# ziwon-park/TRG-planner

Measured on AMD Instinct MI355X. Metric: TRG nodes+edges built/sec, higher is better.
Workload: dtype f32

## Files before the change

### include/trg_engine.h

```cpp
#ifndef TRG_ENGINE_H_
#define TRG_ENGINE_H_

#include <stddef.h>
#include <stdint.h>

#ifdef __cplusplus
extern "C" {
#endif

typedef struct TrgEngine TrgEngine;

typedef enum TrgStatus {
  TRG_OK = 0,
  TRG_ERR_INVALID_ARG = 1,
  TRG_ERR_NO_MAP = 2,
  TRG_ERR_NO_ROOT = 3,
  TRG_ERR_DEVICE = 4,
  TRG_ERR_NO_GRAPH = 5,
  TRG_ERR_NOT_FOUND = 6,
  TRG_ERR_IO = 7,
  TRG_ERR_CAPACITY = 8
} TrgStatus;

typedef enum TrgKind {
// ... 8 lines not shown
typedef struct TrgParams {
  int32_t is_verbose;
  float expand_dist;
  float robot_size;
  int32_t sample_num;
  float height_threshold;
  float collision_threshold;
  float update_collision_threshold;
  float safety_factor;
  float goal_tolerance;
} TrgParams;

typedef struct TrgSampler {
  uint32_t seed;
  int32_t table_bits;
} TrgSampler;

typedef struct TrgCsrView {
  int32_t num_nodes;
  int32_t num_edges;
  const float *node_xyz;
  const int32_t *node_state;
  const int32_t *rowptr;
  const int32_t *col;
  const float *weight;
  const float *dist;
  const int32_t *creation_id;
} TrgCsrView;

typedef struct TrgPathInfo {
  float direct_dist;
  float path_length;
  float avg_risk;
  int32_t num_points;
} TrgPathInfo;

typedef struct TrgStats {
  uint64_t map_points;
  uint64_t expanded_nodes;
  uint64_t trials;
  uint64_t samples;
  uint64_t created_nodes;
  uint64_t invalid_nodes;
  uint64_t edge_calls;
  uint64_t edge_evals_gpu;
  uint64_t nn_ties;
  uint64_t gate_uncertain;
  uint64_t sync_batches;
  uint64_t bytes_sample_kernel;
  uint64_t bytes_spec_kernel;
  uint64_t bytes_edge_kernel;
  uint64_t bytes_index_build;
  double ms_index_build;
  double ms_sample_kernel;
  double ms_spec_kernel;
  double ms_edge_kernel;
  uint64_t launches_sample_kernel;
  uint64_t launches_spec_kernel;
  uint64_t launches_edge_kernel;
  double ms_set_map_total;
  double ms_init_graph_total;
  double ms_replay_host;
  double ms_finalize_host;
  double ms_wait_gpu;
  uint64_t bfs_levels;
  uint64_t used_device_bfs;
  uint64_t bfs_fallbacks;
  uint64_t bfs_max_spin;
  uint64_t bfs_host_levels;
  uint64_t map_nn_ties;
  double ms_bfs_loop;
  double ms_deferred;
  uint64_t map_nn_resolved;
  uint64_t map_nn_unresolved;
  uint64_t bfs_tie_fixups;
  uint64_t bytes_spec_created;
  double ms_rare_events;
  uint64_t bfs_ticket_reruns;
  uint64_t bfs_multipass_rows;
  double ms_upload;
  uint64_t presampled_nodes;
  uint64_t stitch_gate_retries;
  uint64_t stitch_regrows;
} TrgStats;

TrgStatus trg_engine_create(const TrgParams *params, int device, TrgEngine **out);
void trg_engine_destroy(TrgEngine *e);
const char *trg_engine_last_error(const TrgEngine *e);
const char *trg_engine_device_arch(const TrgEngine *e);

TrgStatus trg_engine_set_global_map(TrgEngine *e, const float *xyz, size_t n, size_t stride);
TrgStatus trg_engine_set_global_map_device(TrgEngine *e, const float *d_xyz, size_t n, size_t stride);
TrgStatus trg_engine_set_local_map(TrgEngine *e, const float start_xy[2], const float *xyz, size_t n,
                                   size_t stride);
TrgStatus trg_engine_reset_map(TrgEngine *e, TrgKind kind);
TrgStatus trg_engine_reset_graph(TrgEngine *e, TrgKind kind);

TrgStatus trg_engine_init_graph(TrgEngine *e, const float start_xyz[3], const TrgSampler *sampler);
TrgStatus trg_engine_update_graph(TrgEngine *e);

TrgStatus trg_engine_export_csr(TrgEngine *e, TrgKind kind, TrgCsrView *out);
TrgStatus trg_engine_graph_sizes(TrgEngine *e, TrgKind kind, int32_t *num_nodes, int32_t *num_edges);
TrgStatus trg_engine_save_json(TrgEngine *e, const char *path);
TrgStatus trg_engine_load_json(TrgEngine *e, const char *path);

TrgStatus trg_engine_plan(TrgEngine *e, const float start_xy[2], const float goal_xyz[3],
                          float *path_xyz, int32_t max_points, TrgPathInfo *info);
TrgStatus trg_engine_plan_batch(TrgEngine *e, const float *starts_xy, const float *goals_xyz,
                                size_t m, float *path_xyz, int32_t path_cap, int32_t *offsets,
                                TrgPathInfo *infos);
int32_t trg_engine_check_reached(TrgEngine *e, const float pos_xy[2]);
int32_t trg_engine_check_replan(TrgEngine *e, const float pos_xy[2], const float *path_xyz,
                                int32_t n_path);
int32_t trg_engine_refine_path(const float *in_xyz, int32_t n_in, float *out_xyz, int32_t max_out);

TrgStatus trg_engine_is_collision_batch(TrgEngine *e, TrgKind map, float threshold, const float *xy,
                                        size_t m, int32_t *flag, int32_t *cnt, int32_t *n);
TrgStatus trg_engine_nearest_z_batch(TrgEngine *e, TrgKind map, const float *xy, size_t m, float *z);
TrgStatus trg_engine_edge_risk_batch(TrgEngine *e, TrgKind map, const float *p1_xyz,
                                     const float *p2_xyz, size_t m, int32_t *status, int32_t *n_pts,
                                     float *weight, float *dist);
TrgStatus trg_engine_is_frontier_batch(TrgEngine *e, const float *xy, size_t m, int32_t *flag);
typedef struct TrgPoseInfo {
  int32_t status, n_candidates, n_links;
  float z;
} TrgPoseInfo;
TrgStatus trg_engine_pose_links(TrgEngine *e, const float *poses_xy, int32_t m, float radius, int32_t cap,
                                int32_t *link_node, float *link_weight, float *link_dist, TrgPoseInfo *infos);

TrgStatus trg_engine_voxel_filter(TrgEngine *e, const float *xyz, size_t n, size_t stride, float leaf,
                                  float *out_xyz, size_t *n_out, int32_t *passthrough);

TrgStatus trg_engine_set_option(TrgEngine *e, const char *key, const char *value);
TrgStatus trg_engine_set_tile(TrgEngine *e, const float core_xyxy[4], uint32_t epoch);
typedef struct TrgBoundaryRec { int32_t local_id; float x, y, z; } TrgBoundaryRec;
typedef struct TrgCrossEdge { int32_t tile_a, id_a, tile_b, id_b; float weight, dist; } TrgCrossEdge;
TrgStatus trg_engine_stitch_boundary(TrgEngine *e, const float core_xyxy[4], int32_t cols, int32_t rows,
                                     int32_t tile, TrgBoundaryRec *d_rec, int32_t cap, int32_t *n_out);
TrgStatus trg_engine_stitch_cross(TrgEngine *e, int32_t tile, int32_t ntiles, const TrgBoundaryRec *d_all_rec,
                                  const int32_t *rec_offsets, TrgCrossEdge *d_edges, int32_t cap,
                                  int32_t *n_out);
TrgStatus trg_engine_stitch_assemble(TrgEngine *e, int32_t tile, int32_t ntiles, const int32_t *node_offsets,
                                     const TrgCrossEdge *d_all_edges, int32_t n_edges);
#define TRG_COMM_ID_BYTES 128
TrgStatus trg_engine_comm_unique_id(TrgEngine *e, uint8_t id[TRG_COMM_ID_BYTES]);
TrgStatus trg_engine_comm_init(TrgEngine *e, const uint8_t id[TRG_COMM_ID_BYTES], int32_t nranks, int32_t rank);
TrgStatus trg_engine_comm_adopt(TrgEngine *e, void *nccl_comm);
TrgStatus trg_engine_comm_join_local(TrgEngine *e, const char *group_name, int32_t nranks, int32_t rank);
TrgStatus trg_engine_comm_destroy(TrgEngine *e);
TrgStatus trg_engine_stitch_exchange(TrgEngine *e, const float core_xyxy[4], int32_t cols, int32_t rows,
                                     int32_t *n_boundary, int32_t *n_cross);
const char *trg_engine_fallback_reason(const TrgEngine *e);

typedef struct TrgFieldInfo {
  int32_t source;
  int32_t reached;
  int32_t rounds;
  int32_t host_syncs;
  double ms_device;
  double ms_total;
} TrgFieldInfo;
TrgStatus trg_engine_cost_field(TrgEngine *e, int32_t source_id, const float source_xy[2],
                                float *cost, int32_t *hops, int32_t *parent, TrgFieldInfo *info);
#define TRG_FIELD_BATCH_MAX 64
TrgStatus trg_engine_cost_field_batch(
    TrgEngine *e, int32_t m,
// ... 113 lines not shown
```

### trg-planner_amd/csrc/trg_bfs.inc

```

__device__ __forceinline__ int bfs_cell_x(const BfsDev &B, float x) {
  float t = floorf((x - B.gx0) * B.ginv);
  t = fminf(fmaxf(t, 0.0f), (float)(B.GW - 1));
  return (int)t;
}
__device__ __forceinline__ int bfs_cell_y(const BfsDev &B, float y) {
  float t = floorf((y - B.gy0) * B.ginv);
  t = fminf(fmaxf(t, 0.0f), (float)(B.GH - 1));
  return (int)t;
}
__device__ __forceinline__ float bfs_d2(float nx, float ny, float qx, float qy) {
  float acc = 0.0f;
  acc += (nx - qx) * (nx - qx);
  acc += (ny - qy) * (ny - qy);
  return acc;
}
__device__ __forceinline__ uint32_t bfs_hash(int key) { return fmix32((uint32_t)key * 0x9E3779B1u); }

__global__ __launch_bounds__(256) void k_bfs_insert_nodes(BfsDev B, int first, int count) {
  const int i = blockIdx.x * blockDim.x + threadIdx.x;
  if (i >= count) return;
  const int id = first + i;
  GridCell &c = B.gcell[bfs_cell_y(B, B.ny[id]) * B.GW + bfs_cell_x(B, B.nx[id])];
  const int pos = atomicAdd(&c.cnt, 1);
  if (pos < GRID_SLOTS) {
    c.id[pos] = id;
    c.x[pos] = B.nx[id];
    c.y[pos] = B.ny[id];
  } else {
    atomicOr(&B.ctrs[BFS_CTR_ERR], BFS_ERR_GRID_OVERFLOW);
  }
}

__device__ __forceinline__ int outcome_load(const int *p) {
  return __hip_atomic_load(p, __ATOMIC_RELAXED, __HIP_MEMORY_SCOPE_AGENT);
}
__device__ __forceinline__ void outcome_store(int *p, int v) {
  __hip_atomic_store(p, v, __ATOMIC_RELAXED, __HIP_MEMORY_SCOPE_AGENT);
}

#ifndef SPEC_WAVES_PER_SIMD
#define SPEC_WAVES_PER_SIMD 6
#endif
#ifndef SPEC3_WAVES_PER_SIMD
#define SPEC3_WAVES_PER_SIMD 5
#endif
#ifndef RESOLVE_EARLY_CREATE
#define RESOLVE_EARLY_CREATE 1
#endif
#ifndef TRG_RWV
#define TRG_RWV 8
#endif
constexpr int RW = TRG_RWV * 4;
static_assert(256 % RW == 0, "a commit workgroup covers whole resolve groups");

__global__ void k_bfs_clear_tie(BfsDev B) {
  if (threadIdx.x == 0) {
    atomicAnd(&B.ctrs[BFS_CTR_ERR], ~BFS_ERR_TIE);
    B.ctrs[BFS_CTR_NTIE] = 0;
  }
}

__global__ __launch_bounds__(256) void k_bfs_undo_slots(BfsDev B, int slots) {
  if (blockIdx.x == 0 && threadIdx.x == 0) B.stats64[STATS64_EXPAND_START] = 0ull;
  const int slot = blockIdx.x * blockDim.x + threadIdx.x;
  if (slot >= slots) return;
  const int o = B.c_outcome[slot];
  if (o != 3 && o != 4) return;
  const SlotRec &sr = B.slot_rec[slot];
  if ((sr.cls & SLOT_CLS_MASK) != 2) return;
  atomicSub(&B.gcell[bfs_cell_y(B, sr.y) * B.GW + bfs_cell_x(B, sr.x)].cnt, 1);
}

__global__ __launch_bounds__(QW *WAVE, EDGE_WAVES_PER_SIMD) void k_calls_gather(MapView m, QueryParams p, BfsDev B,
                                                           const int *list, int count,
                                                           const int *count_dev, DeviceCounters *ctr) {
  __shared__ EdgeLds lds;
  const int w = threadIdx.x >> 6;
  const int q = blockIdx.x * QW + w;
  if (count_dev) count = min(count, *count_dev);
  if (q >= count) return;
  const size_t at = (size_t)list[q];
  if (B.call_status[at] != CALL_PENDING) return;
  const int a = B.call_n1[at], b = B.call_n2[at];
  float *rec = B.mid + (size_t)q * MID_STRIDE;
  const EdgeMidOut o = edge_gather(m, p, B.nx[a], B.ny[a], B.nz[a], B.nx[b], B.ny[b], B.nz[b],
                                   lds.w[w], rec, ctr);
  store_mid(rec, o);
}

__global__ __launch_bounds__(256) void k_calls_finish(BfsDev B, const int *list, int count,
                                                      const int *count_dev, DeviceCounters *ctr) {
  __shared__ int wave_hits[4];
  const int q = blockIdx.x * blockDim.x + threadIdx.x;
  if (count_dev) count = min(count, *count_dev);
  const size_t at = (size_t)list[q < count ? q : 0];
  const bool live = q < count && B.call_status[at] == CALL_PENDING;
  const float *r = B.mid + (size_t)(live ? q : 0) * MID_STRIDE;
  const int h = wave_sum(live ? __float_as_int(r[MID_HITS]) : 0);
  if (lane_id() == 0) wave_hits[threadIdx.x >> 6] = h;
  __syncthreads();
  if (threadIdx.x == 0 && ctr) {
    const unsigned long long tot =
        (unsigned long long)(wave_hits[0] + wave_hits[1] + wave_hits[2] + wave_hits[3]);
    if (tot) atomicAdd(&ctr[blockIdx.x % COUNTER_SHARDS].edge_hits, tot);
  }
  if (!live) return;
  int st = __float_as_int(r[0]);
  float w = 0.0f;
  if ((st & EDGE_STATUS_MASK) == EDGE_OK) {
    float cov[3][3];
    mid_covariance(r, cov);
    int clamped = 0;
    w = risk_weight(cov, clamped);
    st |= clamped;
  }
  if (st & EDGE_GATE_UNCERTAIN) {
    const int k = atomicAdd(&B.ctrs[BFS_CTR_NUNC2], 1);
    if (k < BFS_UNC_CAP) {
      const int u = 2 * BFS_UNC_CAP + k;
      B.unc_list[u] = (int)at;
      B.unc_rec[3 * u] = B.nz[B.call_n1[at]];
      B.unc_rec[3 * u + 1] = B.nz[B.call_n2[at]];
      B.unc_rec[3 * u + 2] = r[2];
    }
  }
  B.call_status[at] = st & (EDGE_STATUS_MASK | EDGE_CLAMPED | EDGE_GATE_UNCERTAIN);
  B.call_w[at] = w;
  B.call_dist[at] = r[2];
}

__device__ __forceinline__ unsigned long long pair_key(int a, int b) {
  const unsigned lo = (unsigned)min(a, b), hi = (unsigned)max(a, b);
  return ((unsigned long long)lo << 32) | hi;
}
__device__ __forceinline__ uint32_t hash64(unsigned long long k) {
  return fmix32((uint32_t)(k >> 32) * 0x85EBCA6Bu ^ fmix32((uint32_t)k));
}

__global__ __launch_bounds__(256) void k_first_insert(FinDev F, BfsDev B, long long c0, long long ncalls,
                                                      int *sel_count) {
  if (blockIdx.x == 0 && threadIdx.x == 0) *sel_count = 0;
  const long long i = c0 + (long long)blockIdx.x * blockDim.x + threadIdx.x;
  if (i >= ncalls) return;
  F.call_slot[i] = -1;
  if (B.call_status[i] == CALL_NONE) return;
  int n2 = B.call_n2[i];
  if (n2 <= -2) {
    n2 = B.newid_of_call[-(long long)n2 - 2];
    B.call_n2[i] = n2;
  }
  const unsigned long long key = pair_key(B.call_n1[i], n2);
  const uint32_t mask = F.ht_size - 1u;
  uint32_t s = hash64(key) & mask;
  for (uint32_t probe = 0; probe < F.ht_size; ++probe) {
    const unsigned long long prev = atomicCAS(&F.ht_key[s], ~0ull, key);
    if (prev == ~0ull || prev == key) {
      atomicMin(&F.ht_seq[s], (int)i);
      F.call_slot[i] = (int)s;
      return;
    }
    s = (s + 1) & mask;
  }
  atomicOr(&B.ctrs[BFS_CTR_ERR], BFS_ERR_HASH);
}

__global__ __launch_bounds__(256) void k_calls_select_append(FinDev F, BfsDev B, long long c0, long long ncalls,
                                                             int *list, int *count, unsigned long long *total) {
  __shared__ int wave_cnt[4];
  __shared__ int wg_base;
  const long long i = c0 + (long long)blockIdx.x * blockDim.x + threadIdx.x;
  bool sel = false;
  if (i < ncalls && B.call_status[i] == CALL_PENDING) {
    const int slot = F.call_slot[i];
    sel = slot >= 0 && F.ht_seq[slot] == (int)i;
  }
  const unsigned long long m = ballot(sel);
  const int w = threadIdx.x >> 6;
  if (lane_id() == 0) wave_cnt[w] = __popcll(m);
  __syncthreads();
  if (threadIdx.x == 0) {
    const int tot = wave_cnt[0] + wave_cnt[1] + wave_cnt[2] + wave_cnt[3];
    if (tot) {
      wg_base = atomicAdd(count, tot);
      if (total) atomicAdd(total, (unsigned long long)tot);
    }
  }
  __syncthreads();
  if (!sel) return;
  int rank = __popcll(m & lanemask_lt());
  for (int k = 0; k < w; ++k) rank += wave_cnt[k];
// ... 205 lines not shown
```

### trg-planner_amd/csrc/trg_engine.cpp

```cpp
#include <hip/hip_runtime.h>
#include <math.h>

#include <algorithm>
#include <array>
#include <atomic>
#include <cstddef>
#include <chrono>
#include <cstdio>
#include <cstring>
#include <deque>
#include <fstream>
#include <functional>
#include <memory>
#include <optional>
#include <queue>
#include <sstream>
#include <string>
#include <thread>
#include <unordered_map>
#include <vector>

#include "../../include/trg_engine.h"
#include "abi_frame.h"
#include "graph_json.h"
// ... 435 lines not shown
struct TrgEngine {
  TrgEngine();
  ~TrgEngine();
  TrgParams prm{};
  int device = 0;
  int wall_clock_khz = 0;
  std::string err;
  std::string arch;
  bool device_ok = false;

  Stream s_main, s_edge;
  Stream s_aux;
  DevBuf<float> top_xy_d;
  Pinned<float> top_xy_h;
  Event top_ev;
  DevMap gmap, lmap;
  IndexScratch idx_scratch;
  DevBuf<DeviceCounters> d_ctr;
  DevBuf<unsigned> d_bounds;

  TrgSampler sampler{1, 16};
  std::vector<float> cos_t, sin_t;
  DevBuf<float> d_cos, d_sin;
  int table_bits_dev = 0;
  uint32_t epoch = 0;
  uint32_t epoch_base = 0;
  float core[4] = {-INFINITY, -INFINITY, INFINITY, INFINITY};

  enum GraphView { VIEW_POOL, VIEW_GRID, VIEW_KD_ORDER, VIEW_KD, VIEW_KDO, VIEW_CSR, VIEW_DEV_CSR, VIEW_UP_NODES,
                   VIEW_UP_EDGES, VIEW_STITCH_DEV, VIEW_COUNT };
  uint64_t graph_version = 1;
  uint64_t view_stamp[VIEW_COUNT] = {};
  bool current(GraphView v) const { return view_stamp[v] == graph_version; }
  std::vector<float> nx, ny, nz;
  std::vector<int> nstate;
  std::vector<int> ncid;
  int next_cid = 0;
  int node_id = 0;
  std::unordered_map<int, int> order_map;
  MapOrderSim nodes_sim;
  bool history_in_sim = false;
  std::vector<int> last_new2old;
  EdgePool edges;
  NodeGrid grid;
  std::vector<int> kd_insert_order;
  NodeKd kd;
  std::vector<float> kdo_x, kdo_y;
  std::vector<int> kdo_index;
  Csr csr_global;
  DevGraphUpload dev_up;
  Csr csr_stitched;
  int stitched_edges = 0;
  std::vector<int32_t> stitch_node_off;
  int stitch_tile = -1;
  uint64_t stitch_serial = 0;
  float root_pos[2] = {0, 0};
  float local_root[2] = {0, 0};
  std::unordered_map<int, int> local_map;
  std::vector<int> local_nodes;
  bool step3 = false;

  std::vector<int> queue;
  std::vector<CallRec> calls;
  static constexpr int NCHUNK = 3;
  static constexpr int CHUNK_MAX = 4096;
  Chunk chunks[NCHUNK];
  Chunk root_chunk;
  static constexpr int NEBATCH = 3;
  static constexpr int EBATCH_MAX = 1 << 16;
  EdgeBatch ebatches[NEBATCH];
  std::vector<int> pending_calls;

  PinnedBuf<float> sy_in, sy_in2, sy_f0, sy_f1;
  PinnedBuf<int> sy_i0, sy_i1, sy_i2;
  DevBuf<float> sy_mid;
  PinnedBuf<MapTieSet> mt_set;
  PinnedBuf<MapTieWalk> mt_walk;

  Csr csr_pre, csr_local;
  std::unique_ptr<StitchBufs> stitch;
  bool keep_preclean = false;
  bool use_device_bfs = true;
  bool defer_overlap = true;
  bool tail_overlap = true;
  PlanScratch plan_scratch;
  std::unique_ptr<Uploader> uploader;
  std::unique_ptr<ExchangeState> exchange;
  std::unique_ptr<FieldBufs> field;
  std::unique_ptr<TiledFieldBufs> tiled;
  double field_delta_scale = 4.0;
  enum { FIELD_MAP_NONE, FIELD_MAP_IDENTITY, FIELD_MAP_EXPLICIT } field_map_state = FIELD_MAP_NONE;
  std::vector<int> field_map;
  int debug_tie_every = 0;
  int debug_spec_bound = 0;
  int debug_fallback_level = -1;
  bool tie_inplace = true;
  int debug_lookback_level = -1;
  int debug_stall_level = -1;
  bool debug_wait_rerun = false;
  bool debug_call_stride = false;
  int resolve_tickets = 0;
  float gate_margin = 1e-4f;
  int debug_stitch_cap = 0;
  double comm_wait_seconds = 20.0;
  std::unique_ptr<BfsBuffers> bfs;
  std::string bfs_fallback_reason;
  uint64_t lv_hits_sample = 0, lv_hits_spec = 0;
  TrgStats stats{};

  int goal_node = -1;
  bool goal_known = false;
  float goal_pose2d[2] = {0, 0};

  TrgStatus fail(TrgStatus s, const std::string &m) {
    err = m;
    return s;
  }
};

namespace {

#define HIPCHK(e, expr)                                                                   \
  do {                                                                                    \
    hipError_t _err = (expr);                                                             \
    if (_err != hipSuccess) {                                                             \
      return (e)->fail(TRG_ERR_DEVICE, std::string(#expr) + ": " + hipGetErrorString(_err)); \
    }                                                                                     \
  } while (0)

enum EntryNeed { ENGINE, DEVICE };
template <typename Body>
TrgStatus entry(TrgEngine *e, const char *call, EntryNeed need, Body body) {
  if (!e) return TRG_ERR_INVALID_ARG;
  return abi_guard(call, [e](TrgStatus s, const std::string &m) { return e->fail(s, m); }, [&]() -> TrgStatus {
    if (need == DEVICE) {
      if (!e->device_ok) return e->fail(TRG_ERR_DEVICE, "engine has no usable device");
      if (hipSetDevice(e->device) != hipSuccess) return e->fail(TRG_ERR_DEVICE, "hipSetDevice failed");
    }
    return body();
  });
}

TrgStatus ensure_bytes(TrgEngine *e, DevArr &a, size_t need, bool keep = false) {
  if (a.p && a.bytes >= need) return TRG_OK;
  DevArr grown;
  HIPCHK(e, grown.reserve(std::max(need, a.bytes + a.bytes / 2)));
  if (keep && a.p && a.bytes) {
    hipError_t he = hipMemcpy(grown.p, a.p, a.bytes, hipMemcpyDeviceToDevice);
    if (he != hipSuccess) return e->fail(TRG_ERR_DEVICE, std::string("grow copy: ") + hipGetErrorString(he));
  }
  std::swap(a, grown);
  return TRG_OK;
}
TrgStatus ensure_all(TrgEngine *e, std::initializer_list<std::pair<DevArr *, size_t>> need) {
  for (const auto &n : need) {
    const TrgStatus st = ensure_bytes(e, *n.first, n.second);
    if (st != TRG_OK) return st;
  }
  return TRG_OK;
}

QueryParams qparams(const TrgEngine *e) {
  QueryParams q;
  q.robot_size = e->prm.robot_size;
  q.height_threshold = e->prm.height_threshold;
  q.collision_threshold = e->prm.collision_threshold;
  q.expand_dist = e->prm.expand_dist;
  q.sample_num = e->prm.sample_num;
  q.core_x0 = e->core[0];
  q.core_y0 = e->core[1];
  q.core_x1 = e->core[2];
  q.core_y1 = e->core[3];
  q.gate_margin = e->gate_margin;
  return q;
}

inline float key_to_float(unsigned k) {
  unsigned b = (k & 0x80000000u) ? (k & 0x7FFFFFFFu) : ~k;
  float f;
  memcpy(&f, &b, 4);
  return f;
}

#include "trg_engine_map.ipp"

TrgStatus ensure_sampler(TrgEngine *e, const TrgSampler *smp) {
  TrgSampler want = smp ? *smp : e->sampler;
  if (want.table_bits < 2 || want.table_bits > 20) want.table_bits = 16;
  e->sampler = want;
  if (e->table_bits_dev == want.table_bits && e->d_cos) return TRG_OK;
// ... 276 lines not shown
  if (e->arch.rfind("gfx950", 0) != 0) {
    return e->fail(TRG_ERR_DEVICE, "kernels are built for gfx950 only, device is " + e->arch);
  }
  HIPCHK(e, hipDeviceGetAttribute(&e->wall_clock_khz, hipDeviceAttributeWallClockRate, device));
  if (e->wall_clock_khz <= 0) return e->fail(TRG_ERR_DEVICE, "the device reports no wall-clock rate");
  HIPCHK(e, e->s_main.create());
  HIPCHK(e, e->s_edge.create_with_priority(0));
  HIPCHK(e, e->s_aux.create());
  HIPCHK(e, e->d_ctr.ensure(COUNTER_SHARDS));
  HIPCHK(e, hipMemset(e->d_ctr, 0, COUNTER_SHARDS * sizeof(DeviceCounters)));
  HIPCHK(e, e->d_bounds.ensure(4));
  e->step3 = (e->prm.expand_dist - e->prm.robot_size) < 0.25 * e->prm.expand_dist;
  e->bfs.reset(new BfsBuffers());
  e->uploader.reset(new Uploader());
  e->device_ok = true;
  if (const char *env = getenv("TRG_REPLAY")) e->use_device_bfs = std::string(env) != "host";
  reset_graph_global(e);
  return TRG_OK;
}

TrgStatus set_global_map(TrgEngine *e, const float *xyz, size_t n, size_t stride) {
  if ((n && !xyz) || stride < 3) return e->fail(TRG_ERR_INVALID_ARG, "bad map arguments");
  auto t0 = Clock::now();
  TrgStatus st = upload_and_build(e, e->gmap, xyz, n, stride);
  e->stats.ms_set_map_total = ms_since(t0);
  return st;
}

TrgStatus set_global_map_device(TrgEngine *e, const float *d_xyz, size_t n, size_t stride) {
  if ((n && !d_xyz) || stride < 3) return e->fail(TRG_ERR_INVALID_ARG, "bad map arguments");
  if (n == 0) {
    e->gmap.n = 0;
    e->gmap.valid = false;
    return TRG_OK;
  }
  return build_map(e, e->gmap, d_xyz, n, stride);
}

TrgStatus set_local_map(TrgEngine *e, const float start_xy[2], const float *xyz, size_t n, size_t stride) {
  if (!start_xy || (n && !xyz) || stride < 3) return e->fail(TRG_ERR_INVALID_ARG, "bad arguments");
  e->local_root[0] = start_xy[0];
  e->local_root[1] = start_xy[1];
  TrgStatus st = upload_and_build(e, e->lmap, xyz, n, stride);
  if (st != TRG_OK) return st;
  return set_local_graph(e);
}

TrgStatus reset_map(TrgEngine *e, TrgKind kind) {
  DevMap *m = pick_map(e, kind);
  m->top_wait();
  m->n = 0;
  m->valid = false;
  return TRG_OK;
}

TrgStatus reset_graph(TrgEngine *e, TrgKind kind) {
  if (kind == TRG_KIND_LOCAL) {
    e->local_nodes.clear();
    e->local_map.clear();
  } else {
    ensure_real_map(e);
    reset_graph_global(e);
    e->csr_global.clear();
    field_release(e);
  }
  return TRG_OK;
}

TrgStatus init_graph(TrgEngine *e, const float start_xyz[3], const TrgSampler *sampler) {
  if (!start_xyz) return e->fail(TRG_ERR_INVALID_ARG, "null start");
  if (!e->gmap.valid || e->gmap.n == 0) return e->fail(TRG_ERR_NO_MAP, "Map is empty");
  auto t_total = Clock::now();
  TrgStatus st = ensure_sampler(e, sampler);
  if (st != TRG_OK) return st;
  {
    TrgStats keep = e->stats;
    e->stats = TrgStats();
    e->stats.map_points = keep.map_points;
    e->stats.ms_index_build = keep.ms_index_build;
    e->stats.bytes_index_build = keep.bytes_index_build;
    e->stats.ms_set_map_total = keep.ms_set_map_total;
  }
  HIPCHK(e, hipMemsetAsync(e->d_ctr, 0, COUNTER_SHARDS * sizeof(DeviceCounters), e->s_main));
  e->lv_hits_sample = e->lv_hits_spec = 0;
  if (!e->use_device_bfs) ensure_real_map(e);
  MapOrderSim sim_before;
  if (e->use_device_bfs) {
    if (!e->history_in_sim) e->nodes_sim.adopt_bucket_state(e->order_map);
    sim_before = e->nodes_sim;
  }
  reset_graph_global(e);
  e->epoch = e->epoch_base;
  e->calls.clear();
  e->pending_calls.clear();
  e->csr_pre.clear();

  e->root_pos[0] = start_xyz[0];
  e->root_pos[1] = start_xyz[1];
  float rx = e->root_pos[0], ry = e->root_pos[1], rz = 0.0f;
  rx = rx + e->prm.expand_dist;
  int cnt = 0;
  for (;;) {
    float xy[2] = {rx, ry};
    int32_t flag = 1;
    st = collision_sync(e, e->gmap, e->prm.collision_threshold, xy, 1, &flag, nullptr, nullptr);
    if (st != TRG_OK) return st;
    if (!(rx >= e->core[0] && rx < e->core[2] && ry >= e->core[1] && ry < e->core[3])) flag = 1;
    if (!flag) {
      int32_t found = 0;
      st = nearest_z_sync(e, e->gmap, xy, 1, &rz, &found);
      if (st != TRG_OK) return st;
      break;
    }
    if (cnt > 100) return e->fail(TRG_ERR_NO_ROOT, "Failed to generate root node");
    const float u0 = sampler_uniform(e, 2 * cnt), u1 = sampler_uniform(e, 2 * cnt + 1);
    rx = rx + e->prm.expand_dist * u0;
    ry = ry + e->prm.expand_dist * u1;
    cnt++;
  }

  if (e->use_device_bfs) {
    st = build_graph_device(e, rx, ry, rz);
    if (st == TRG_OK) {
      read_counters(e);
      e->stats.used_device_bfs = 1;
      e->stats.ms_init_graph_total = ms_since(t_total);
      return TRG_OK;
    }
    if (e->bfs_fallback_reason.empty()) return st;
    e->stats.bfs_fallbacks++;
    HIPCHK(e, hipStreamSynchronize(e->s_main));
    HIPCHK(e, hipStreamSynchronize(e->s_edge));
    HIPCHK(e, hipMemset(e->d_ctr, 0, COUNTER_SHARDS * sizeof(DeviceCounters)));
    e->lv_hits_sample = e->lv_hits_spec = 0;
    e->nodes_sim = sim_before;
    ensure_real_map(e);
    reset_graph_global(e);
  }

  grid_rebuild(e);
  add_node_host(e, rx, ry, rz, TRG_NODE_VALID);
  st = expand_bfs(e, e->node_id - 1);
  if (st != TRG_OK) return st;
  auto t_fin = Clock::now();
  st = flush_pending(e, true);
  if (st != TRG_OK) return st;
  apply_calls(e, 0);
  if (e->keep_preclean) snapshot_csr(e, e->csr_pre);
  clean_graph(e);
  host_graph_changed(e);
  e->stats.ms_finalize_host = ms_since(t_fin);
  read_counters(e);
  e->stats.ms_init_graph_total = ms_since(t_total);
  return TRG_OK;
}

TrgStatus set_option(TrgEngine *e, const char *key, const char *value) {
  enum Kind {
    INT,
    BOOL,
    ZERO_OR_ONE,
    HOST_OR_DEVICE,
    FLOAT,
    POSITIVE_DOUBLE
  };
  const struct {
    const char *name;
    Kind kind;
    void *target;
  } options[] = {
      {"replay", HOST_OR_DEVICE, &e->use_device_bfs},
      {"defer_overlap", ZERO_OR_ONE, &e->defer_overlap},
      {"tail_overlap", ZERO_OR_ONE, &e->tail_overlap},
      {"tie_inplace", BOOL, &e->tie_inplace},
      {"keep_preclean", BOOL, &e->keep_preclean},
      {"resolve_tickets", INT, &e->resolve_tickets},
      {"field_delta_scale", POSITIVE_DOUBLE, &e->field_delta_scale},
      {"debug_gate_margin", FLOAT, &e->gate_margin},
      {"debug_tie_every", INT, &e->debug_tie_every},
      {"debug_spec_bound", INT, &e->debug_spec_bound},
      {"debug_stall_level", INT, &e->debug_stall_level},
      {"debug_lookback_level", INT, &e->debug_lookback_level},
      {"debug_fallback_level", INT, &e->debug_fallback_level},
      {"debug_call_stride", BOOL, &e->debug_call_stride},
      {"debug_wait_rerun", BOOL, &e->debug_wait_rerun},
      {"debug_stitch_cap", INT, &e->debug_stitch_cap},
      {"comm_wait_seconds", POSITIVE_DOUBLE, &e->comm_wait_seconds},
  };
  const std::string k(key), v(value);
  for (const auto &o : options) {
    if (k != o.name) continue;
    switch (o.kind) {
      case INT:
        *(int *)o.target = atoi(value);
        break;
      case BOOL:
        *(bool *)o.target = v != "0";
        break;
      case ZERO_OR_ONE:
        if (v != "0" && v != "1") return e->fail(TRG_ERR_INVALID_ARG, k + " must be 0 or 1");
        *(bool *)o.target = v == "1";
        break;
      case HOST_OR_DEVICE:
        if (v != "host" && v != "device") return e->fail(TRG_ERR_INVALID_ARG, k + " must be host or device");
        *(bool *)o.target = v == "device";
        break;
      case FLOAT:
        *(float *)o.target = (float)atof(value);
        break;
      case POSITIVE_DOUBLE: {
        const double d = strtod(value, nullptr);
        if (!(d > 0.0)) return e->fail(TRG_ERR_INVALID_ARG, k + " must be > 0");
        *(double *)o.target = d;
        break;
      }
    }
    return TRG_OK;
  }
  return e->fail(TRG_ERR_INVALID_ARG, "unknown option " + k);
}

TrgStatus set_tile(TrgEngine *e, const float core_xyxy[4], uint32_t epoch) {
  if (core_xyxy) {
    for (int i = 0; i < 4; ++i) e->core[i] = core_xyxy[i];
  } else {
    e->core[0] = e->core[1] = -INFINITY;
    e->core[2] = e->core[3] = INFINITY;
  }
  e->epoch_base = epoch;
  return TRG_OK;
}

TrgStatus is_frontier_batch(TrgEngine *e, const float *xy, size_t m, int32_t *flag);

TrgStatus update_graph(TrgEngine *e) {
  if (!e->gmap.valid) return e->fail(TRG_ERR_NO_MAP, "Map is empty");
  TrgStatus st = ensure_sampler(e, nullptr);
  if (st != TRG_OK) return st;
  e->epoch++;
  e->view_stamp[TrgEngine::VIEW_DEV_CSR] = 0;
  const size_t nodes_before = e->nx.size();
  const auto map_before = e->field_map_state;
  e->field_map_state = TrgEngine::FIELD_MAP_NONE;
  const bool trace_up = getenv("TRG_TIMING") != nullptr;
  auto t_up = Clock::now();
  auto lap_up = [&](const char *what) {
    if (trace_up) fprintf(stderr, "[trg update] %-28s %8.3f ms\n", what, ms_since(t_up));
  };
  ensure_pool(e);
  ensure_host_grid(e);
  ensure_kd_order(e);
  e->calls.clear();
  e->pending_calls.clear();
  lap_up("host structures ready");

  const size_t L = e->local_nodes.size();
// ... 512 lines not shown
```

### trg-planner_amd/csrc/trg_engine_bfs.inc

```

namespace {

struct LevelSet {
  DevArr node_rec;
  DevArr slot_rec;
  DevArr c_outcome;
  DevArr lv_hash;
  DevArr resc;
  void apply(BfsDev &B) const {
    B.node_rec = (NodeRec *)node_rec.p;
    B.slot_rec = (SlotRec *)slot_rec.p;
    B.c_outcome = (int *)c_outcome.p;
    B.lv_hash = (HashEnt *)lv_hash.p;
    B.resc = use_resc ? (RescueRec *)resc.p : nullptr;
  }
  bool use_resc = false;
};

constexpr int H_CLEAN_TOTALS = 32;
constexpr int H_ROUND2_CALLS = 34;
constexpr int H_STEP3_LEFT = 40;
constexpr int H_STATS64 = 64;
constexpr int H_CTRS_WORDS = 96;
static_assert(BFS_CTR_COUNT <= H_CLEAN_TOTALS && H_CLEAN_TOTALS + 2 <= H_ROUND2_CALLS &&
                  H_ROUND2_CALLS < H_STEP3_LEFT && H_STEP3_LEFT < H_STATS64 && H_STATS64 % 2 == 0 &&
                  H_STATS64 + 32 <= H_CTRS_WORDS,
              "pinned words overlap");

enum : int {
  S64_DEF_KEPT = 5, S64_MAX_SPIN, S64_MULTIPASS, S64_DRAWS, S64_SAMPLES, S64_DISC_HITS, S64_SPEC_HITS,
  S64_CANDIDATES, S64_PARENT_HITS, S64_EXPAND_START = STATS64_EXPAND_START, S64_EXPAND_TICKS = STATS64_EXPAND_TICKS,
  S64_PHASES = 16, S64_WORDS = 16 + 1024 * 8
};
static_assert(S64_PARENT_HITS < S64_EXPAND_START && S64_EXPAND_START < S64_EXPAND_TICKS && S64_EXPAND_TICKS < S64_PHASES,
              "report_stats fetches the words in front of S64_PHASES");

struct BfsBuffers {
  BfsDev B{};
  FinDev F{};
  LevelSet lv[2];
  DevArr nx, ny, nz, nstate, gcell, ncov, nexp, nhits, front0, front1, fxy0, fxy1;
  DevArr mid, unc_list, unc_rec, mt_rec, ctrs, stats64, wg_state, c_cell, tl, scan_tmp, s3_scratch;
  DevArr call_n1, call_n2, call_status, call_w, call_dist, newid_of_call, call_slot;
  DevArr sel_list, def_counts;
  DevArr ht_key, ht_seq, ok_seq, deg, fill, rowptr, col, seq, w, dist;
  DevArr map_order, keep_flag, keep_pos, new2old, old2new, deg_new, rowptr_new, col2, w2, dist2, xyz2, state2;
  Pinned<int> h_ctrs;
  int stamp_serial = 0;
  std::vector<int> hm_state;
  std::vector<float> hm_x, hm_y;
  std::vector<int> rp_stamp, rp_head;
  int rp_serial = 0;
  unsigned long long nodes_created = 0, nodes_invalid = 0;
};

TrgStatus mirror_nodes(TrgEngine *e, BfsBuffers &bb, int n) {
  const size_t at = bb.hm_state.size();
  if ((size_t)n <= at) return TRG_OK;
  const size_t k = (size_t)n - at;
  bb.hm_state.resize(n);
  bb.hm_x.resize(n);
  bb.hm_y.resize(n);
  HIPCHK(e, hipMemcpy(bb.hm_state.data() + at, bb.B.nstate + at, k * sizeof(int), hipMemcpyDeviceToHost));
  HIPCHK(e, hipMemcpy(bb.hm_x.data() + at, bb.B.nx + at, k * sizeof(float), hipMemcpyDeviceToHost));
  HIPCHK(e, hipMemcpy(bb.hm_y.data() + at, bb.B.ny + at, k * sizeof(float), hipMemcpyDeviceToHost));
  return TRG_OK;
}

inline float ref_d2(float x, float y, float qx, float qy) {
  float acc = 0;
  acc += (x - qx) * (x - qx);
  acc += (y - qy) * (y - qy);
  return acc;
}

struct Nearest {
  int nn = -1;
  float best = INFINITY;
  std::vector<int> tied;
  void start(const BfsBuffers &bb, const SlotRec &sr, int V0) {
    nn = sr.nn0;
    best = nn >= 0 ? sr.d0sq : INFINITY;
    tied.clear();
    if (nn >= 0 && (sr.cls & SLOT_TIE)) {
      for (int i = 0; i < V0; ++i)
        if (ref_d2(bb.hm_x[i], bb.hm_y[i], sr.x, sr.y) == best) tied.push_back(i);
    } else if (nn >= 0) {
      tied.push_back(nn);
    }
  }
  void offer(const BfsBuffers &bb, int id, float qx, float qy) {
    const float dd = ref_d2(bb.hm_x[id], bb.hm_y[id], qx, qy);
    if (dd < best) {
      best = dd;
      nn = id;
      tied.assign(1, id);
    } else if (dd == best) {
      tied.push_back(id);
    }
  }
  bool tie() const { return tied.size() > 1; }
  int winner(const BfsBuffers &bb, int V_at, float qx, float qy) {
    if (!tie()) return nn;
    std::sort(tied.begin(), tied.end());
    return kd_tie_winner(bb.hm_x.data(), bb.hm_y.data(), V_at, qx, qy, tied);
  }
};

constexpr int BFS_FCAP = 1 << 16;
constexpr int CALL_EVAL_BATCH = 1 << 22;
constexpr int BFS_ERR_SOFT = BFS_ERR_TIE | BFS_ERR_STALL | BFS_ERR_TIE_CLS;
constexpr long long DEF_BATCH_MIN = 6000;

std::string err_text(int code) {
  std::string t;
  if (code & BFS_ERR_GRID_OVERFLOW) t += "grid-cell overflow;";
  if (code & BFS_ERR_NB_OVERFLOW) t += "neighbour list overflow;";
  if (code & BFS_ERR_VCAP) t += "node capacity;";
  if (code & BFS_ERR_TIE) t += "exact fp32 distance tie (kd-tree order decides);";
  if (code & BFS_ERR_TIE_CLS) t += "exact fp32 distance tie among pre-level nodes;";
  if (code & BFS_ERR_HASH) t += "hash table full;";
  if (code & BFS_ERR_LEVEL_TOO_BIG) t += "BFS level too large;";
  if (code & BFS_ERR_CLEAN) t += "clean remap;";
  if (code & BFS_ERR_STALL) t += "resolve stalled;";
// ... 344 lines not shown
    float t = std::floor((v - v0) * B.ginv);
    t = std::min(std::max(t, 0.0f), (float)(n - 1));
    return (int)t;
  };
  std::vector<int> call_n1(slots), call_n2(slots, -1), call_st(slots, CALL_NONE), next_front;
  std::vector<float> call_w(slots, 0.0f), call_d(slots, 0.0f);
  Nearest near;
  int Vcur = V0;
  unsigned long long invalid = 0;
  for (int qpos = 0; qpos < lv.mcur; ++qpos) {
    const int u = front[qpos];
    for (int j = 0; j < S; ++j) {
      const size_t slot = (size_t)qpos * S + j;
      call_n1[slot] = u;
      if (j >= nrec[qpos].n_acc) continue;
      const SlotRec &sr = srec[slot];
      const float qx = sr.x, qy = sr.y;
      near.start(bb, sr, V0);
      {
        const float rad = (near.nn >= 0 ? std::sqrt(near.best) : e->prm.expand_dist * 1.01f) * 1.001f + 1e-6f;
        const int cx0 = cell_xy(qx - rad, B.gx0, B.GW), cx1 = cell_xy(qx + rad, B.gx0, B.GW);
        const int cy0 = cell_xy(qy - rad, B.gy0, B.GH), cy1 = cell_xy(qy + rad, B.gy0, B.GH);
        for (int cy = cy0; cy <= cy1; ++cy)
          for (int cx = cx0; cx <= cx1; ++cx) {
            const size_t cell = (size_t)cy * B.GW + cx;
            if (bb.rp_stamp[cell] != serial) continue;
            for (int id = bb.rp_head[cell]; id >= 0; id = rp_next[id - V0]) near.offer(bb, id, qx, qy);
          }
      }
      if (near.nn < 0) return e->fail(TRG_ERR_DEVICE, "host level replay: a sample without a nearest node");
      if (near.tie()) e->stats.nn_ties++;
      const int nn = near.winner(bb, Vcur, qx, qy);
      if (bb.hm_state[nn] == TRG_NODE_INVALID) continue;
      if (std::sqrt(near.best) < e->prm.robot_size) {
        if (nn != u) {
          call_n2[slot] = nn;
          call_st[slot] = CALL_PENDING;
        }
        continue;
      }
      if ((sr.cls & SLOT_CLS_MASK) != 2)
        return e->fail(TRG_ERR_DEVICE, "host level replay: missing speculative edge");
      const bool ok = (sr.status & EDGE_STATUS_MASK) == EDGE_OK;
      const int id = Vcur++;
      new_hits.push_back(sr.hits);
      bb.hm_x.push_back(qx);
      bb.hm_y.push_back(qy);
      bb.hm_state.push_back(ok ? TRG_NODE_VALID : TRG_NODE_INVALID);
      new_z.push_back(sr.z);
      {
        const size_t cell = (size_t)cell_xy(qy, B.gy0, B.GH) * B.GW + cell_xy(qx, B.gx0, B.GW);
        rp_next.push_back(bb.rp_stamp[cell] == serial ? bb.rp_head[cell] : -1);
        bb.rp_stamp[cell] = serial;
        bb.rp_head[cell] = id;
      }
      NodeCov nc{};
      if (ok) {
        call_n2[slot] = id;
        call_st[slot] = sr.status & EDGE_STATUS_MASK;
        call_d[slot] = sr.dist;
        next_front.push_back(id);
        if (sr.w_given) nc.cov[0] = sr.cov[0];
        nc.w_given = sr.w_given;
        nc.call = (int)(lv.call_base + (long long)slot);
      } else {
        invalid++;
      }
      new_cov.push_back(nc);
    }
  }
  const int created = Vcur - V0;
  bb.nodes_created += (unsigned long long)created;
  bb.nodes_invalid += invalid;
  if (Vcur > B.vcap || (int)next_front.size() > B.fcap)
    return e->fail(TRG_ERR_CAPACITY, "host level replay: capacity");
  if (created > 0) {
    const size_t at = (size_t)V0, n = (size_t)created;
    HIPCHK(e, hipMemcpy(B.nx + at, bb.hm_x.data() + at, n * sizeof(float), hipMemcpyHostToDevice));
    HIPCHK(e, hipMemcpy(B.ny + at, bb.hm_y.data() + at, n * sizeof(float), hipMemcpyHostToDevice));
    HIPCHK(e, hipMemcpy(B.nz + at, new_z.data(), n * sizeof(float), hipMemcpyHostToDevice));
    HIPCHK(e, hipMemcpy(B.nstate + at, bb.hm_state.data() + at, n * sizeof(int), hipMemcpyHostToDevice));
    HIPCHK(e, hipMemcpy(B.ncov + at, new_cov.data(), n * sizeof(NodeCov), hipMemcpyHostToDevice));
    HIPCHK(e, hipMemcpy(B.nhits + at, new_hits.data(), n * sizeof(int), hipMemcpyHostToDevice));
    launch_bfs_insert_nodes(B, V0, created, s);
  }
  if (!next_front.empty()) {
    HIPCHK(e, hipMemcpy(B.front_next, next_front.data(), next_front.size() * sizeof(int),
                        hipMemcpyHostToDevice));
    std::vector<float> fxy(2 * next_front.size());
    for (size_t k = 0; k < next_front.size(); ++k) {
      fxy[2 * k] = bb.hm_x[next_front[k]];
      fxy[2 * k + 1] = bb.hm_y[next_front[k]];
    }
    HIPCHK(e, hipMemcpy(B.fxy_next, fxy.data(), fxy.size() * sizeof(float), hipMemcpyHostToDevice));
  }
  const size_t cb = (size_t)lv.call_base;
  HIPCHK(e, hipMemcpy(B.call_n1 + cb, call_n1.data(), slots * sizeof(int), hipMemcpyHostToDevice));
  HIPCHK(e, hipMemcpy(B.call_n2 + cb, call_n2.data(), slots * sizeof(int), hipMemcpyHostToDevice));
  HIPCHK(e, hipMemcpy(B.call_status + cb, call_st.data(), slots * sizeof(int), hipMemcpyHostToDevice));
  HIPCHK(e, hipMemcpy(B.call_w + cb, call_w.data(), slots * sizeof(float), hipMemcpyHostToDevice));
  HIPCHK(e, hipMemcpy(B.call_dist + cb, call_d.data(), slots * sizeof(float), hipMemcpyHostToDevice));
  int ctr_host[BFS_CTR_COUNT] = {0};
  ctr_host[BFS_CTR_V] = Vcur;
  ctr_host[BFS_CTR_MNEXT] = (int)next_front.size();
  HIPCHK(e, hipMemcpy(B.ctrs, ctr_host, BFS_CTR_NUNC2 * sizeof(int), hipMemcpyHostToDevice));
  HIPCHK(e, hipStreamSynchronize(s));
  lv.v_after = Vcur;
  lv.mnext = (int)next_front.size();
  lv.replayed = true;
  e->stats.bfs_host_levels++;
  return TRG_OK;
}

TrgStatus Build::repair_level(Level &lv) {
  TrgStatus st;
  if (e->step3 && lv.n_unc > 0)
    return fallback("a slope gate left to the host's libm in a build with expandGraph's step 3");
  if (CS > 1 && ((lv.err & BFS_ERR_SOFT & ~BFS_ERR_STALL) || lv.n_mt > 0))
    return fallback("exact fp32 distance tie in a build with expandGraph's step 3");
  const auto t_rare = Clock::now();
  const bool any_rare = lv.n_mt > 0 || lv.n_unc > 0 || (lv.err & (BFS_ERR_SOFT | BFS_ERR_LOOKBACK));
  constexpr int ERR_WAIT = BFS_ERR_STALL | BFS_ERR_LOOKBACK;
  if ((lv.err & ERR_WAIT) && !(lv.err & ~(BFS_ERR_SOFT | ERR_WAIT))) {
    const int hook = e->debug_wait_rerun ? ((lv.err & BFS_ERR_LOOKBACK) ? 2 : 1) : 0;
    e->stats.bfs_ticket_reruns++;
    st = redo_commit(lv, false, true, hook);
    if (st == TRG_ERR_CAPACITY) e->stats.ms_rare_events += ms_since(t_rare);
    if (st != TRG_OK) return st;
  }
  if (lv.err & ~BFS_ERR_SOFT) {
    if (any_rare) e->stats.ms_rare_events += ms_since(t_rare);
    return fallback(err_text(lv.err));
  }
  if (lv.n_mt > 0 && (st = fix_map_ties(lv)) != TRG_OK) return st;
  if (lv.n_unc > 0) {
    void *status = (char *)B.slot_rec + offsetof(SlotRec, status);
    if ((st = resolve_uncertain(lv.n_unc, status, sizeof(SlotRec), lv.parity, lv.unc_ctr)) != TRG_OK) return st;
    if (unc_changed && (st = (lv.err & BFS_ERR_SOFT) ? undo_level(lv) : redo_commit(lv)) != TRG_OK) return st;
  }
  if ((lv.err & BFS_ERR_SOFT) == BFS_ERR_TIE_CLS && !lv.undone && (st = fix_pre_level_ties(lv)) != TRG_OK)
    return st;
  if ((lv.err & BFS_ERR_SOFT) == BFS_ERR_TIE && !lv.undone && e->tie_inplace && !debug_tie_level(e, lv.index)) {
    if ((st = settle_ties_in_place(lv)) != TRG_OK) return st;
  }
  if (lv.err & BFS_ERR_SOFT) {
    if (CS > 1) return fallback("a level of a build with expandGraph's step 3 needs the host replay");
    if (!lv.undone && (st = undo_level(lv)) != TRG_OK) return st;
    if ((st = replay_level(lv)) != TRG_OK) return st;
  }
  if (any_rare) {
    e->stats.ms_rare_events += ms_since(t_rare);
    if (getenv("TRG_TRACE_LEVELS"))
      fprintf(stderr, "[trg bfs] level %d: rare events (map ties %d, uncertain gates %d, err %d%s) took %.3f ms\n",
              lv.index, lv.n_mt, lv.n_unc, lv.err, lv.replayed ? ", host replay" : "",
              ms_since(t_rare));
  }
  return TRG_OK;
}

TrgStatus Build::allocate() {
  const float pad = e->prm.expand_dist * 2 + e->prm.robot_size;
  float cell = e->prm.robot_size;
  if (!(cell > 0)) return fallback("robot_size <= 0");
  const double ex = (double)(m.bounds[2] - m.bounds[0]) + 2 * pad + 4 * cell;
  const double ey = (double)(m.bounds[3] - m.bounds[1]) + 2 * pad + 4 * cell;
  if ((ex / cell + 2) * (ey / cell + 2) > 256e6) return fallback("node grid too large");
  B.gx0 = m.bounds[0] - pad - 2 * cell;
  B.gy0 = m.bounds[1] - pad - 2 * cell;
  B.gcell_size = cell;
  B.ginv = 1.0f / cell;
  B.GW = (int)floor(ex / cell) + 2;
  B.GH = (int)floor(ey / cell) + 2;
  const size_t ncell = (size_t)B.GW * B.GH;
  const double vbound = ex * ey / (0.8660254 * cell * cell) * 1.05 + 4096;
  if (vbound > 400e6) return fallback("node capacity bound too large");
  const size_t vcap = (size_t)vbound;
  const size_t fcap = BFS_FCAP;
  const size_t slots = fcap * (size_t)std::max(S, 1);

  if (!level_kernels_support(qp, cell))
    return fallback("sample_num or expand_dist / robot_size outside the level kernels' range");
  TrgStatus st;
  const size_t wg_words = slots / 16 + 64 + 8;
  const size_t I = sizeof(int), FL = sizeof(float);
  if ((st = ensure_all(e, {{&bb.nx, vcap * FL}, {&bb.ny, vcap * FL}, {&bb.nz, vcap * FL}, {&bb.nstate, vcap * I},
                           {&bb.gcell, ncell * sizeof(GridCell)}, {&bb.ncov, vcap * sizeof(NodeCov)},
                           {&bb.front0, fcap * I}, {&bb.front1, fcap * I}, {&bb.fxy0, fcap * sizeof(float2)},
                           {&bb.fxy1, fcap * sizeof(float2)}})) != TRG_OK)
    return st;
  B.nx = (float *)bb.nx.p;
  B.ny = (float *)bb.ny.p;
  B.nz = (float *)bb.nz.p;
  B.nstate = (int *)bb.nstate.p;
  B.vcap = (int)std::min<size_t>(vcap, 0x7FFFFFF0);
  B.gcell = (GridCell *)bb.gcell.p;
  B.ncov = (NodeCov *)bb.ncov.p;
  B.front_cur = (int *)bb.front0.p;
  B.front_next = (int *)bb.front1.p;
  B.fxy_cur = (float2 *)bb.fxy0.p;
  B.fxy_next = (float2 *)bb.fxy1.p;
  B.fcap = (int)fcap;
  const size_t ht_need = hash_size(fcap, std::max(S, 1));
  for (LevelSet &l : bb.lv) {
    if ((st = ensure_all(e, {{&l.node_rec, fcap * sizeof(NodeRec)}, {&l.slot_rec, slots * sizeof(SlotRec)},
                             {&l.c_outcome, slots * I}, {&l.lv_hash, ht_need * sizeof(HashEnt)}})) != TRG_OK)
      return st;
    l.use_resc = e->step3;
    if (e->step3 && (st = ensure_bytes(e, l.resc, slots * sizeof(RescueRec))) != TRG_OK) return st;
    HIPCHK(e, hipMemsetAsync(l.lv_hash.p, 0, ht_need * sizeof(HashEnt), s));
  }
  if ((st = ensure_all(e, {{&bb.mid, edge_mid_floats(CALL_EVAL_BATCH) * FL},
                           {&bb.unc_list, (3 * BFS_UNC_CAP + BFS_TIE_CAP) * I},
                           {&bb.unc_rec, 3 * 3 * BFS_UNC_CAP * FL}, {&bb.mt_rec, 2 * MAPTIE_CAP * sizeof(MapTieRec)},
                           {&bb.ctrs, BFS_CTR_COUNT * I}, {&bb.stats64, S64_WORDS * sizeof(unsigned long long)},
                           {&bb.wg_state, wg_words * sizeof(unsigned long long)},
                           {&bb.c_cell, slots * sizeof(unsigned long long)}, {&bb.nexp, vcap * sizeof(int4)},
                           {&bb.nhits, vcap * I}, {&bb.scan_tmp, (std::max(slots, vcap) / 2048 + 8) * I}})) != TRG_OK)
    return st;
  B.mid = (float *)bb.mid.p;
  B.unc_list = (int *)bb.unc_list.p;
  B.tie_list = B.unc_list + 3 * BFS_UNC_CAP;
  B.unc_rec = (float *)bb.unc_rec.p;
  B.mt_rec = (MapTieRec *)bb.mt_rec.p;
  B.ctrs = (int *)bb.ctrs.p;
  B.stats64 = (unsigned long long *)bb.stats64.p;
  B.wg_state = (unsigned long long *)bb.wg_state.p;
  HIPCHK(e, hipMemsetAsync(B.wg_state, 0, wg_words * sizeof(unsigned long long), s));
  B.ticket = (unsigned *)(B.wg_state + (slots / 16 + 64));
  ticket_base = 0;
  B.tl = nullptr;
  if (getenv("TRG_TIMELINE")) {
    const size_t tl_bytes = (size_t)(1 << 16) * 12 * 6 * sizeof(unsigned long long);
    if ((st = ensure_bytes(e, bb.tl, tl_bytes)) != TRG_OK) return st;
    B.tl = (unsigned long long *)bb.tl.p;
    HIPCHK(e, hipMemsetAsync(B.tl, 0, tl_bytes, s));
  }
  B.c_cell = (unsigned long long *)bb.c_cell.p;
  HIPCHK(e, hipMemsetAsync(B.c_cell, 0, slots * sizeof(unsigned long long), s));
  B.nexp = (int4 *)bb.nexp.p;
  B.nhits = (int *)bb.nhits.p;
  if (!bb.h_ctrs) {
    HIPCHK(e, bb.h_ctrs.ensure(H_CTRS_WORDS, hipHostMallocMapped | hipHostMallocCoherent));
    memset(bb.h_ctrs, 0, H_CTRS_WORDS * sizeof(int));
  }
  {
    void *dp = nullptr;
    HIPCHK(e, hipHostGetDevicePointer(&dp, bb.h_ctrs, 0));
    B.host_ctrs = (int *)dp;
  }

  bb.hm_state.clear();
  bb.hm_x.clear();
  bb.hm_y.clear();
  bb.nodes_created = bb.nodes_invalid = 0;
  HIPCHK(e, hipMemsetAsync(B.gcell, 0, ncell * sizeof(GridCell), s));
  HIPCHK(e, hipMemsetAsync(B.ctrs, 0, BFS_CTR_COUNT * sizeof(int), s));
  HIPCHK(e, hipMemsetAsync(B.stats64, 0, S64_WORDS * sizeof(unsigned long long), s));

  calls_bound = std::min<size_t>(vcap * (size_t)std::max(S, 1) * (size_t)CS, 0x7FFFFFF0u);
  fht = 1024;
  while ((unsigned long long)fht < (unsigned long long)calls_bound && fht < (1u << 31)) fht <<= 1;
  if ((st = ensure_all(e, {{&bb.ht_key, fht * sizeof(unsigned long long)}, {&bb.ht_seq, fht * I},
                           {&bb.ok_seq, fht * I}, {&bb.def_counts, 2 * I}})) != TRG_OK)
    return st;
  F.ht_key = (unsigned long long *)bb.ht_key.p;
  F.ht_seq = (int *)bb.ht_seq.p;
  F.ok_seq = (int *)bb.ok_seq.p;
  F.ht_size = fht;
  overlap = !e->step3 && e->defer_overlap;
  if (overlap) {
    HIPCHK(e, hipMemsetAsync(F.ht_key, 0xFF, (size_t)fht * sizeof(unsigned long long), s));
    HIPCHK(e, hipMemsetAsync(F.ht_seq, 0x7F, (size_t)fht * sizeof(int), s));
  }
  HIPCHK(e, hipMemsetAsync(F.ok_seq, 0x7F, (size_t)fht * sizeof(int), s));
  s_def = overlap ? e->s_edge : s;
  return TRG_OK;
// ... 370 lines not shown
    if ((st = read_ctrs()) != TRG_OK) return st;
    if (bb.h_ctrs[BFS_CTR_ERR]) return fallback(err_text(bb.h_ctrs[BFS_CTR_ERR]));
    e->nx.clear();
    e->ny.clear();
    e->nz.clear();
    e->nstate.clear();
    e->ncid.clear();
  }
  lap("clean kernels + CSR to host");
  e->node_id = Vn;
  lap("host graph state");
  e->history_in_sim = true;
  if (Vn > 0) graph_changed(e, {TrgEngine::VIEW_CSR, TrgEngine::VIEW_DEV_CSR});
  else graph_changed(e, {TrgEngine::VIEW_CSR});
  return TRG_OK;
}

TrgStatus Build::report_stats() {
  unsigned long long s64[S64_PHASES];
  memcpy(s64, bb.h_ctrs + H_STATS64, sizeof(s64));
  if (getenv("TRG_DEBUG_STATS")) {
    std::vector<int> hs(V), hx(4 * (size_t)V);
    HIPCHK(e, hipMemcpy(hs.data(), B.nstate, (size_t)V * sizeof(int), hipMemcpyDeviceToHost));
    HIPCHK(e, hipMemcpy(hx.data(), B.nexp, (size_t)V * 16, hipMemcpyDeviceToHost));
    unsigned long long d = 0, a = 0;
    size_t zero = 0;
    for (int i = 0; i < V; ++i)
      if (hs[i] != -1) {
        d += (unsigned long long)hx[4 * (size_t)i + 1];
        a += (unsigned long long)(hx[4 * (size_t)i] & 0xFF);
        zero += hx[4 * (size_t)i + 1] == 0;
      }
    fprintf(stderr, "[trg stats] device draws %llu samples %llu | host sum draws %llu samples %llu | valid nodes with 0 draws %zu\n",
            s64[S64_DRAWS], s64[S64_SAMPLES], d, a, zero);
  }
  if (B.tl) {
    constexpr int UNITS = 1 << 16, KINDS = 12, TAGS = 6;
    std::vector<unsigned long long> tl((size_t)UNITS * KINDS * TAGS);
    HIPCHK(e, hipMemcpy(tl.data(), B.tl, tl.size() * sizeof(unsigned long long), hipMemcpyDeviceToHost));
    static const char *names[KINDS] = {"sample start", "sample end", "spec start", "spec end", "resolve start",
                                       "resolve collected", "resolve decided(w0)", "resolve published",
                                       "(unused)", "(unused)", "commit start", "commit sums known"};
    for (int t = 0; t < TAGS; ++t) {
      const unsigned long long *base = &tl[(size_t)t * UNITS * KINDS];
      unsigned long long t0 = ~0ull;
      for (int i = 0; i < UNITS; ++i)
        if (base[i]) t0 = std::min(t0, base[i]);
      if (t0 == ~0ull) continue;
      fprintf(stderr, "[trg timeline] level attempt +%d (us after its first sampling workgroup started; n, min, p10, median, p90, max):\n", t);
      for (int k = 0; k < KINDS; ++k) {
        std::vector<double> v;
        for (int i = 0; i < UNITS; ++i)
          if (base[(size_t)k * UNITS + i]) v.push_back(((double)base[(size_t)k * UNITS + i] - (double)t0) / 100.0);
        if (v.empty()) continue;
        std::sort(v.begin(), v.end());
        auto q = [&](double f) { return v[(size_t)(f * (v.size() - 1))]; };
        fprintf(stderr, "[trg timeline]   %-22s n=%6zu  %8.1f %8.1f %8.1f %8.1f %8.1f%s\n", names[k], v.size(), q(0), q(0.1), q(0.5),
                q(0.9), q(1), k >= 4 ? "   (of the PREVIOUS level's resolve launch)" : "");
      }
    }
  }
  if (getenv("TRG_PHASE_TIMING") && ncalls > 0) {
    std::vector<unsigned long long> ph(1024 * 8);
    HIPCHK(e, hipMemcpy(ph.data(), B.stats64 + S64_PHASES, ph.size() * sizeof(unsigned long long), hipMemcpyDeviceToHost));
    double t[8] = {0};
    for (size_t i = 0; i < ph.size(); ++i) t[i & 7] += (double)ph[i];
    const double nodes = (double)(ncalls / std::max(S * CS, 1));
    if (getenv("TRG_PHASE_TIMING")[0] == 'r')
      fprintf(stderr, "[trg resolve phases, cycles per workgroup] collect %.0f  decide(wave 0) %.0f  records+stash %.0f  other waves %.0f  look-back %.0f\n",
              t[0] / nodes * (32.0 / S), t[1] / nodes * (32.0 / S), t[2] / nodes * (32.0 / S), t[3] / nodes * (32.0 / S), t[4] / nodes * (32.0 / S));
    else
    fprintf(stderr, "[trg expand phases, cycles per node] sample: tile %.0f  nodegrid %.0f  sampling %.0f  classify %.0f  hash %.0f  record %.0f | spec (per node): tile %.0f  edges %.0f\n",
            t[0] / nodes, t[1] / nodes, t[2] / nodes, t[3] / nodes, t[4] / nodes, t[5] / nodes, t[6] / nodes, t[7] / nodes);
  }
  e->stats.expanded_nodes = (uint64_t)(ncalls / std::max(S * CS, 1));
  e->stats.trials = s64[S64_DRAWS];
  e->stats.samples = s64[S64_SAMPLES];
  e->stats.created_nodes = bb.nodes_created + 1;
  e->stats.invalid_nodes = bb.nodes_invalid;
  e->stats.edge_calls = s64[S64_SAMPLES];
  e->stats.edge_evals_gpu = s64[S64_CANDIDATES] + s64[S64_DEF_KEPT];
  e->lv_hits_sample = s64[S64_DISC_HITS];
  e->lv_hits_spec = s64[S64_SPEC_HITS];
  e->stats.bytes_spec_created = 12ull * s64[S64_PARENT_HITS];
  e->stats.ms_finalize_host = ms_since(t_fin);
  e->stats.bfs_levels = (uint64_t)levels;
  e->stats.bfs_max_spin = s64[S64_MAX_SPIN];
  e->stats.ms_sample_kernel += (double)s64[S64_EXPAND_TICKS] / (double)e->wall_clock_khz;
  e->stats.bfs_multipass_rows = s64[S64_MULTIPASS];
  return TRG_OK;
}

TrgStatus build_graph_device(TrgEngine *e, float root_x, float root_y, float root_z) {
  e->bfs_fallback_reason.clear();
  Build b(e);
  b.B.cstride = b.CS;
  TrgStatus st;
  if ((st = b.allocate()) != TRG_OK) return st;
  if ((st = b.seed_root(root_x, root_y, root_z)) != TRG_OK) return st;
  if ((st = b.level_loop()) != TRG_OK) return st;
  if ((st = b.finish_deferred()) != TRG_OK) return st;
  if ((st = b.assemble_csr()) != TRG_OK) return st;
  if ((st = b.clean_and_fetch()) != TRG_OK) return st;
  return b.report_stats();
}

}
```

### trg-planner_amd/csrc/trg_kernels.h

```cpp
#pragma once
#include <hip/hip_runtime.h>
#include <stdint.h>

namespace trg {

struct MapView {
  const float *x;
  const float *y;
  const float *z;
  const int *perm;
  const float4 *pt;
  const int *cell_start;
  float x0, y0;
  float inv_g;
  int W, H;
  int n;
};

constexpr int MAPTIE_CAP = 256;
constexpr int MAPTIE_SET_CAP = 16;
struct MapTieRec {
  int slot;
  float qx, qy;
  float d2;
};
struct MapTieSet {
  int count;
  float d2;
  int sidx[MAPTIE_SET_CAP];
  int perm[MAPTIE_SET_CAP];
  float x[MAPTIE_SET_CAP], y[MAPTIE_SET_CAP], z[MAPTIE_SET_CAP];
};

struct QueryParams {
  float robot_size;
  float height_threshold;
  float collision_threshold;
  float expand_dist;
  int sample_num;
  float core_x0, core_y0, core_x1, core_y1;
  float gate_margin;
};

enum : int {
  EDGE_OK = 0,
  EDGE_GATE = 1,
  EDGE_SEG = 2,
  EDGE_EMPTY = 3,
  EDGE_FEW = 4,
  EDGE_STATUS_MASK = 7,
  EDGE_GATE_UNCERTAIN = 8,
  EDGE_CLAMPED = 16,
};

constexpr int COUNTER_SHARDS = 64;
struct alignas(128) DeviceCounters {
  unsigned long long sample_hits;
  unsigned long long edge_hits;
  unsigned long long spec_hits;
  unsigned long long nn_ties;
  unsigned long long overflow;
  unsigned long long pad[11];
};

void launch_init_bounds(unsigned *d_bounds, hipStream_t s);
void launch_bounds(const float *d_xyz, size_t n, size_t stride, unsigned *d_bounds, hipStream_t s);
void launch_cell_count(const float *d_xyz, size_t n, size_t stride, float x0, float y0, float inv_g,
                       int W, int H, int *d_cell_of, int *d_rank, int *d_counts, hipStream_t s);
hipError_t voxel_grid_filter(const float *d_xyz, size_t n, size_t stride, float leaf, float *d_out,
                             size_t *n_out, int *status, hipStream_t s);
void launch_exclusive_scan(const int *d_counts, int *d_out, int m, int *d_tmp, hipStream_t s);
bool index_bins_plan(size_t n, size_t ncell, int *bin_shift, int *nbins, int *nwg);
void launch_index_bins(const float *d_xyz, size_t n, size_t stride, float x0, float y0, float inv_g, int W, int H,
                       int ncell, int bin_shift, int nbins, int nwg, int *d_hist, int *d_base, int *d_tmp,
                       float4 *d_scratch_a, float4 *d_scratch_b, int *d_cell_start, float *x, float *y, float *z,
                       int *perm, float4 *pt, hipStream_t s);
void launch_scatter_sort_aos(const float *d_xyz, size_t n, size_t stride, const int *d_cell_of,
                             const int *d_rank, int ncell, const int *d_cell_start, void *d_aos, float *x,
                             float *y, float *z, int *perm, float4 *pt, hipStream_t s);

void launch_probe_collision(const MapView &m, QueryParams p, float threshold, const float *d_xy,
                            int count, int *flag, int *cnt, int *n, DeviceCounters *ctr,
                            hipStream_t s);
void launch_probe_nearest_z(const MapView &m, QueryParams p, const float *d_xy, int count, float *z,
                            int *found, DeviceCounters *ctr, hipStream_t s);
void launch_edges(const MapView &m, QueryParams p, const float *d_p1, const float *d_p2, int count,
                  float *mid, int *status, int *n_pts, float *weight, float *dist,
                  DeviceCounters *ctr, hipStream_t s);
size_t edge_mid_floats(size_t edges);

void launch_sample_nodes(const MapView &m, QueryParams p, const float *cos_t, const float *sin_t,
                         int table_bits, uint32_t seed, uint32_t epoch, const float *node_xy,
                         const int *node_id, int count, int *n_acc, int *n_draws, float *sx,
                         float *sy, float *sz, DeviceCounters *ctr, int *mt_count,
                         MapTieRec *mt_rec, hipStream_t s);
void launch_map_tied_set(const MapView &m, float qx, float qy, float r0, MapTieSet *d_out,
                         hipStream_t s);
struct MapTieWalk {
  unsigned long long key;
  float lo[2], hi[2];
  int cur_perm;
  int axis;
  float qx, qy;
  int aperm, bperm;
  float ax, ay, bx, by;
  int done;
  int first;
  int steps;
  int ticket;
};
void launch_map_tie_walk(const MapView &m, MapTieWalk *d_state, int grid_steps, int block_steps, hipStream_t s);
void launch_collect_first(const MapView &m, int M, float *d_out_xy, hipStream_t s);
void launch_spec_edges(const MapView &m, QueryParams p, const float *node_xyz, int count,
                       const int *n_acc, const float *sx, const float *sy, const float *sz,
                       float *mid, int *status, int *n_pts, float *weight, float *dist,
                       DeviceCounters *ctr, hipStream_t s);

constexpr int GRID_SLOTS = 4;
constexpr int BFS_TIE_CAP = 64;
constexpr int BFS_UNC_CAP = 4096;
enum : int {
  BFS_CTR_V = 0, BFS_CTR_MNEXT = 1, BFS_CTR_NCAND = 2, BFS_CTR_NUNC = 3, BFS_CTR_ERR = 4,
  BFS_CTR_DONE = 5,
  BFS_CTR_NTIE = 5,
  BFS_CTR_NMAPTIE = 6 ,
  BFS_CTR_NUNC1 = 8,
  BFS_CTR_NUNC2 = 14,
  BFS_CTR_COUNT = 16
};
enum : int {
  BFS_ERR_GRID_OVERFLOW = 1, BFS_ERR_NB_OVERFLOW = 2, BFS_ERR_VCAP = 4, BFS_ERR_TIE = 8,
  BFS_ERR_HASH = 16, BFS_ERR_LEVEL_TOO_BIG = 32, BFS_ERR_CLEAN = 64,
  BFS_ERR_STALL = 128,
  BFS_ERR_LOOKBACK = 512,
  BFS_ERR_STEP3 = 1024,
  BFS_ERR_TIE_CLS = 256
};
enum : int { CALL_NONE = -2, CALL_PENDING = -1 };

struct alignas(64) GridCell {
  int cnt;
  int id[GRID_SLOTS];
  float x[GRID_SLOTS], y[GRID_SLOTS];
  int pad[3];
};
struct alignas(16) SlotRec {
  float x, y, z;
  float d0sq;
  int nn0;
  int cls;
  int status;
  float dist;
  float cov[6];
  int w_given;
  int hits;
};
enum : int { SLOT_CLS_MASK = 0xFF, SLOT_TIE = 0x100 };
struct alignas(16) NodeRec {
  int n_acc, n_draws;
  int hits_sample, hits_spec;
  unsigned cand_lo, cand_hi;
  int pad1[2];
  float px, py, pz;
  int pad2;
};
struct alignas(16) HashEnt {
  unsigned long long tagcell;
  int slot;
  int pad;
  float x, y;
  int pad2[2];
};
constexpr int RESC_MAX = 14;
struct alignas(16) RescueRec {
  int pre;
  int n;
  int slot[RESC_MAX];
};
struct alignas(16) NodeCov {
  float cov[6];
  int w_given;
  int call;
};

struct BfsDev {
  float *nx, *ny, *nz;
  int *nstate;
  NodeCov *ncov;
  int vcap;
  GridCell *gcell;
  float gx0, gy0, ginv, gcell_size;
  int GW, GH;
  int *front_cur, *front_next;
  float2 *fxy_cur, *fxy_next;
  int fcap;
  NodeRec *node_rec;
  SlotRec *slot_rec;
  int *c_outcome;
  unsigned long long *c_cell;
  HashEnt *lv_hash;
  int ht_size;
  RescueRec *resc;
  unsigned long long *wg_state;
  unsigned *ticket;
  int4 *nexp;
  int *nhits;
  float *mid;
  int *unc_list;
  float *unc_rec;
  int *tie_list;
  MapTieRec *mt_rec;
  int *call_n1, *call_n2, *call_status;
  float *call_w, *call_dist;
  int *newid_of_call;
  int cstride;
  int *ctrs;
  int *host_ctrs;
  unsigned long long *stats64;
  unsigned long long *tl;
};
constexpr int STATS64_EXPAND_START = 14, STATS64_EXPAND_TICKS = 15;

struct FinDev {
  unsigned long long *ht_key;
  int *ht_seq;
  int *ok_seq;
  unsigned ht_size;
  int *call_slot;
  int *deg, *fill, *rowptr;
  int *col, *seq;
  float *w, *dist;
};

void launch_bfs_insert_nodes(const BfsDev &B, int first, int count, hipStream_t s);
void launch_bfs_clear_tie(const BfsDev &B, hipStream_t s);
void launch_bfs_undo_slots(const BfsDev &B, int slots, hipStream_t s);
constexpr int LEVEL_MAX_SAMPLES = 64;
constexpr int LEVEL_STEP3_STRIDE = 16;
void launch_level_expand(const MapView &m, QueryParams p, const float *cos_t, const float *sin_t,
                         int table_bits, uint32_t seed, uint32_t epoch, const BfsDev &B, int count,
                         const int *count_dev, int node_base, int parity, int tag, int pub_stamp,
                         DeviceCounters *ctr, hipStream_t s, int which = 3);
bool level_kernels_support(const QueryParams &p, float grid_cell);
void launch_level_resolve_commit(const BfsDev &B, QueryParams p, int count, int new_state,
                                 long long call_base, int V0, int tag, int epoch, hipStream_t s,
                                 int stall_test,
                                 bool ticketed, unsigned *ticket_base);
typedef int TrgStatus_t;
TrgStatus_t launch_step3_calls(const BfsDev &B, int V, float range, int *scratch, int *h_left, hipStream_t s);
void launch_bfs_stats(const BfsDev &B, int V, unsigned long long *out, hipStream_t s);
void launch_node_cov(const MapView &m, QueryParams p, const BfsDev &B, int v_lo, int v_hi, hipStream_t s);
void launch_node_weights(const BfsDev &B, int V, hipStream_t s);
void launch_calls_eval(const MapView &m, QueryParams p, const BfsDev &B, const int *list, int count,
                       const int *count_dev, DeviceCounters *ctr, hipStream_t s);
void launch_first_insert(const FinDev &F, const BfsDev &B, long long c0, long long c1, int *sel_count,
                         hipStream_t s);
void launch_calls_select_append(const FinDev &F, const BfsDev &B, long long c0, long long c1, int *list,
                                int *count, unsigned long long *total, hipStream_t s);
void launch_calls_select2_append(const FinDev &F, const BfsDev &B, long long ncalls, int *list, int *count,
                                 unsigned long long *total, hipStream_t s);
void launch_fin_insert_count(const FinDev &F, const BfsDev &B, long long ncalls, hipStream_t s);
void launch_fin_scatter(const FinDev &F, const BfsDev &B, long long ncalls, hipStream_t s);
void launch_fin_rowsort(const FinDev &F, int V, hipStream_t s);
void launch_fin_clean(const FinDev &F, const BfsDev &B, const int *map_order, int V, int *keep_flag,
                      int *keep_pos, int *new2old, int *old2new, int *deg_new, int *rowptr_new,
                      int *scan_tmp, int *col, float *w, float *dist, float *xyz, int *state,
                      hipStream_t s);
void launch_fin_clean_weights(const FinDev &F, const BfsDev &B, int V, const int *keep_pos, const int *new2old,
                              const int *rowptr_new, float *w, hipStream_t s);

struct StitchRec {
  int id;
  float x, y, z;
};
struct StitchEdge {
  int tile_a, id_a, tile_b, id_b;
  float weight, dist;
};
constexpr int STITCH_MAX_TILES = 64;
void launch_stitch_boundary(const float *d_xyz, int V, const float core[4], int sides, float d, int *flag,
                            int *off, int *scan_tmp, StitchRec *rec, int cap, hipStream_t s);
void launch_stitch_pairs(const StitchRec *all, const int *rec_offsets, int tile, int ntiles, float d,
                         int pass, int *cnt, const int *off, int *pair_a, int *pair_b, hipStream_t s);
void launch_stitch_pair_points(const StitchRec *all, const int *pair_a, const int *pair_b, int n,
                               float *p1, float *p2, hipStream_t s);
void launch_stitch_edge_select(const StitchRec *all, const int *rec_offsets, int tile, int ntiles,
                               const int *pair_a, const int *pair_b, const int *status,
                               const float *weight, const float *dist, int n, int *flag, int *off,
                               int *scan_tmp, int *n_unc, StitchEdge *out, int cap, hipStream_t s);
void launch_stitch_assemble(const StitchEdge *edges, int n_edges, int tile, int ntiles,
                            const int *node_offsets, const int *rowptr, const int *col, const float *w,
                            const float *dist, int V, int *extra, int *deg, int *rowptr_new,
                            int *scan_tmp, int *fill, int *col_new, float *w_new, float *dist_new,
                            int phase, hipStream_t s);

constexpr unsigned long long FIELD_KEY_NONE = ~0ull;
constexpr unsigned FIELD_EDGE_SKIP = 0xFFFFFFFFu;
constexpr int FIELD_NODE_INVALID = -1;
constexpr int FIELD_MAX_SOURCES = 64;
struct alignas(128) FieldEdgeStats {
  double sum;
  int count;
  int bad;
};
// ... 133 lines not shown
```

### trg-planner_amd/csrc/trg_kernels.hip

```cpp
#include "trg_kernels.h"

#include <float.h>
#include <limits.h>
#include <type_traits>

namespace trg {

namespace {

constexpr int WAVE = 64;
constexpr int HCAP = 1024;

__device__ __forceinline__ int lane_id() { return threadIdx.x & (WAVE - 1); }

__device__ __forceinline__ unsigned long long lanemask_lt() {
  return (1ull << lane_id()) - 1ull;
}

__device__ __forceinline__ unsigned long long ballot(bool pred) {
  return __builtin_amdgcn_ballot_w64(pred);
}

__device__ __forceinline__ void wave_lds_sync() {
  __builtin_amdgcn_fence(__ATOMIC_RELEASE, "wavefront");
// ... 349 lines not shown
        if (q >= p) continue;
        const float threshold = fmaxf(FLT_MIN, precision * max_diag);
        if (fabsf(W[p][q]) > threshold || fabsf(W[q][p]) > threshold) {
          finished = false;
          Rot jl, jr;
          jacobi_2x2(W, p, q, jl, jr);
          rows_rotate(W, p, q, jl);
          cols_rotate(U, p, q, rot_t(jl));
          cols_rotate(W, p, q, jr);
          max_diag = fmaxf(max_diag, fmaxf(fabsf(W[p][p]), fabsf(W[q][q])));
        }
      }
    }
  }
  float sv[3];
#pragma unroll
  for (int i = 0; i < 3; ++i) {
    const float a = fabsf(W[i][i]);
    sv[i] = a;
    if (a != 0.0f) {
      const float sgn = W[i][i] / a;
#pragma unroll
      for (int r = 0; r < 3; ++r) U[r][i] *= sgn;
    }
  }
#pragma unroll
  for (int i = 0; i < 3; ++i) sv[i] *= scale;
#pragma unroll
  for (int i = 0; i < 3; ++i) {
    int pos = i;
    float mx = sv[i];
#pragma unroll
    for (int k2 = 0; k2 < 3; ++k2) {
      if (k2 > i && sv[k2] > mx) {
        mx = sv[k2];
        pos = k2;
      }
    }
    if (mx == 0.0f) break;
    if (pos != i) {
      const float ts = sv[i];
      sv[i] = sv[pos];
      sv[pos] = ts;
#pragma unroll
      for (int r = 0; r < 3; ++r) {
        const float tu = U[r][i];
        U[r][i] = U[r][pos];
        U[r][pos] = tu;
      }
    }
  }
}

__device__ float risk_weight(const float cov[3][3], int &clamped) {
  float U[3][3];
  svd_u3(cov, U);
  float fro = 0.0f;
#pragma unroll
  for (int cc = 0; cc < 3; ++cc)
#pragma unroll
    for (int r = 0; r < 3; ++r) fro += U[r][cc] * U[r][cc];
  float e20 = U[2][0], e21 = U[2][1];
  if (fro > 0.0f) {
    const float nrm = sqrtf(fro);
    e20 = e20 / nrm;
    e21 = e21 / nrm;
  }
  float hor = e20, ver = e21;
  if (hor < 0.0f) hor = -e20;
  if (ver < 0.0f) ver = -e21;
  const float ratio = 0.8f;
  float w = ratio * hor + (1 - ratio) * ver;
  clamped = 0;
  if ((double)w < 0.1) {
    w = 0.0f;
    clamped = EDGE_CLAMPED;
  }
  return w;
}

constexpr int MID_STRIDE = 24;
constexpr int MID_HITS = 3;
constexpr int MID_MOMENTS = 4;

struct EdgeGeom {
  float dist, dirx, diry, cx, cy;
  int uncertain;
  bool gated;
};

__device__ __forceinline__ EdgeGeom edge_geometry(const QueryParams &p, float x1, float y1, float z1,
                                                  float x2, float y2, float z2) {
  EdgeGeom g;
  const float ex = x1 - x2, ey = y1 - y2;
  g.dist = sqrtf(ex * ex + ey * ey);
  g.uncertain = 0;
  g.gated = false;
  const double lhs = (double)fabsf(z1 - z2) * (double)p.robot_size;
  const double rhs = (double)p.height_threshold * (double)g.dist;
  const double margin = (double)p.gate_margin;
  if (lhs > rhs * (1.0 + margin)) {
    g.gated = true;
  } else if (!(lhs < rhs * (1.0 - margin))) {
    g.uncertain = EDGE_GATE_UNCERTAIN;
  }
  const float dx = x2 - x1, dy = y2 - y1;
  const float sq = dx * dx + dy * dy;
  g.dirx = dx;
  g.diry = dy;
  if (sq > 0.0f) {
    const float nrm = sqrtf(sq);
    g.dirx = dx / nrm;
    g.diry = dy / nrm;
  }
  const float half = 0.5f * g.dist;
  g.cx = x1 + half * g.dirx;
  g.cy = y1 + half * g.diry;
  return g;
}

struct Moments {
  double s_x = 0, s_y = 0, s_z = 0, s_xx = 0, s_xy = 0, s_xz = 0, s_yy = 0, s_yz = 0, s_zz = 0;
  int kept = 0, in_range = 0;
};

struct EllipseParams {
  float cx, cy, a2, bb, aabb, r00, r01, r10, r11, z_ref;
  bool is_circle;
};

__device__ __forceinline__ bool ellipse_point(const EllipseParams &ep, float px, float py, float pz,
                                              Moments &mo) {
  const float ddx = px - ep.cx, ddy = py - ep.cy;
  const float d2 = ddx * ddx + ddy * ddy;
  bool keep = false;
  if (d2 <= ep.a2) {
    mo.in_range++;
    const float X = ep.r00 * ddx + ep.r01 * ddy;
    const float Y = ep.r10 * ddx + ep.r11 * ddy;
    keep = ep.is_circle;
    if (!ep.is_circle) keep = (X * X) * ep.bb + (Y * Y) * ep.a2 < ep.aabb;
    if (keep) {
      mo.kept++;
      const double xd = (double)X, yd = (double)Y, zd = (double)pz - (double)ep.z_ref;
      mo.s_x += xd;
      mo.s_y += yd;
      mo.s_z += zd;
      mo.s_xx += xd * xd;
      mo.s_xy += xd * yd;
      mo.s_xz += xd * zd;
      mo.s_yy += yd * yd;
      mo.s_yz += yd * zd;
      mo.s_zz += zd * zd;
    }
  }
  return keep;
}

struct EllipseCounts {
  int kept = 0, in_range = 0;
};
__device__ __forceinline__ bool ellipse_point(const EllipseParams &ep, float px, float py, float ,
                                              EllipseCounts &mo) {
  const float ddx = px - ep.cx, ddy = py - ep.cy;
  const float d2 = ddx * ddx + ddy * ddy;
  bool keep = false;
// ... 243 lines not shown
  cov[1][2] = cov[2][1] = (float)((sm[7] - n * my * mz) * inv);
  cov[2][2] = (float)((sm[8] - n * mz * mz) * inv);
}

__device__ __forceinline__ void reduce_store_moments(WaveTile &t, const Moments &mo, float *rec) {
  const int lane = lane_id();
  double *P = (double *)&t;
  wave_lds_sync();
  P[0 * MOM_STRIDE + lane] = mo.s_x;
  P[1 * MOM_STRIDE + lane] = mo.s_y;
  P[2 * MOM_STRIDE + lane] = mo.s_z;
  P[3 * MOM_STRIDE + lane] = mo.s_xx;
  P[4 * MOM_STRIDE + lane] = mo.s_xy;
  P[5 * MOM_STRIDE + lane] = mo.s_xz;
  P[6 * MOM_STRIDE + lane] = mo.s_yy;
  P[7 * MOM_STRIDE + lane] = mo.s_yz;
  P[8 * MOM_STRIDE + lane] = mo.s_zz;
  wave_lds_sync();
  const int q = lane / 7, part = lane - q * 7;
  double acc = 0.0;
  if (lane < 63) {
    const double *row = P + q * MOM_STRIDE + part * 10;
    const int cnt = (part == 6) ? 4 : 10;
    int idx = q % cnt;
#pragma unroll
    for (int j = 0; j < 10; ++j)
      if (j < cnt) {
        acc += row[idx];
        idx = (idx + 1 == cnt) ? 0 : idx + 1;
      }
  }
  double *Q = P + 9 * MOM_STRIDE;
  wave_lds_sync();
  if (lane < 63) Q[lane] = acc;
  wave_lds_sync();
  if (lane < 9) {
    double tot = 0.0;
#pragma unroll
    for (int j = 0; j < 7; ++j) tot += Q[lane * 7 + j];
    ((double *)(rec + MID_MOMENTS))[lane] = tot;
  }
}

#ifndef TRG_EDGE_STAGE_CUT
#define TRG_EDGE_STAGE_CUT 0
#endif
#define EDGE_CUT(n)                                \
  if (TRG_EDGE_STAGE_CUT == (n)) {                 \
    o.status = EDGE_SEG;                           \
    return o;                                      \
  }

constexpr int KMAX = 6;

template <int K>
__device__ __forceinline__ void sweep_discs(const WaveTile &tile, int T, const f2 (&q)[KMAX], float r2,
                                            int (&cnt)[KMAX], unsigned (&kmn)[KMAX],
                                            unsigned (&kmx)[KMAX]) {
  const int lane = lane_id();
  for (int base = 0; base < T; base += WAVE) {
    const int i = base + lane;
    const bool valid = i < T;
    const int ii = valid ? i : 0;
    const f2 p = tile.xy[ii];
    const unsigned zk = float_key(tile.z[ii]);
#pragma unroll
    for (int k = 0; k < K; ++k) {
      const f2 d = p - q[k];
      const f2 dd = d * d;
      const float d2 = dd.x + dd.y;
      const bool hit = valid && d2 <= r2;
      cnt[k] += __popcll(ballot(hit));
      const unsigned lo = hit ? zk : 0xFFFFFFFFu, hi = hit ? zk : 0u;
      kmn[k] = lo < kmn[k] ? lo : kmn[k];
      kmx[k] = hi > kmx[k] ? hi : kmx[k];
    }
  }
}

enum : int { GATHER_FULL = 0, GATHER_STATUS = 1, GATHER_MOMENTS = 2 };
template <int MODE = GATHER_FULL>
__device__ EdgeMidOut edge_gather(const MapView &m, const QueryParams &p, float x1, float y1,
                                  float z1, float x2, float y2, float z2, WaveTile &tile,
                                  float *rec, DeviceCounters *ctr) {
  const int lane = lane_id();
  EdgeMidOut o;
  o.n_pts = 0;
  o.hits = 0;
  const EdgeGeom g = edge_geometry(p, x1, y1, z1, x2, y2, z2);
  o.dist = g.dist;
  if (MODE != GATHER_MOMENTS && g.gated) {
    o.status = EDGE_GATE;
    return o;
  }

  const float c = 0.5f * g.dist;
  const float b = p.robot_size;
  float a = b;
  if (c >= b) a = sqrtf(c * c + b * b);
  EllipseParams ep;
  ep.cx = g.cx;
  ep.cy = g.cy;
  ep.is_circle = (a == b);
  ep.r00 = g.dirx;
  ep.r01 = -g.diry;
  ep.r10 = g.diry;
  ep.r11 = g.dirx;
  ep.a2 = a * a;
  ep.bb = b * b;
  ep.aabb = a * a * b * b;
  ep.z_ref = z1;

  CellRange box;
  {
    const float rp = p.robot_size * 1.001f + 1e-6f;
    const float ap = a * 1.001f + 1e-6f;
    const float xlo = fminf(fminf(x1, x2) - rp, g.cx - ap), xhi = fmaxf(fmaxf(x1, x2) + rp, g.cx + ap);
    const float ylo = fminf(fminf(y1, y2) - rp, g.cy - ap), yhi = fmaxf(fmaxf(y1, y2) + rp, g.cy + ap);
    box.cx0 = cell_coord(xlo, m.x0, m.inv_g, m.W);
    box.cx1 = cell_coord(xhi, m.x0, m.inv_g, m.W);
    box.cy0 = cell_coord(ylo, m.y0, m.inv_g, m.H);
    box.cy1 = cell_coord(yhi, m.y0, m.inv_g, m.H);
  }
  CapsuleFilter cf;
  cf.x1 = x1;
  cf.y1 = y1;
  cf.dirx = g.dirx;
  cf.diry = g.diry;
  {
    const float rw = p.robot_size * 1.001f + 1e-3f;
    cf.t_lo = -rw;
    cf.t_hi = g.dist + rw;
    cf.u_max = rw;
  }
  cf.cx = ep.cx;
  cf.cy = ep.cy;
  cf.a2 = ep.a2;
  EDGE_CUT(1)
  int staged_in_range = 0;
  const int T = stage_tile(m, box, tile, cf, staged_in_range);
  if (TRG_EDGE_STAGE_CUT == 2) {
    o.status = EDGE_SEG + (T + staged_in_range > 1000000) +
               (tile.z[lane] + tile.xy[lane].x + tile.xy[lane + 64].y == 12345.0f);
    return o;
  }

  unsigned long long hits = 0;
  const float ds = p.robot_size * 0.5f;
  typedef typename std::conditional<MODE == GATHER_STATUS, EllipseCounts, Moments>::type Gathered;

  if (MODE != GATHER_MOMENTS && T >= 0 && ds > 0.0f) {
    f2 q[KMAX];
    int K = 0;
    bool fits = true;
#pragma unroll
    for (int k = 0; k < KMAX; ++k) q[k] = f2{0.0f, 0.0f};
    for (float i = 0; i < g.dist; i += ds) {
      if (K == KMAX) {
        fits = false;
        break;
      }
#pragma unroll
      for (int k = 0; k < KMAX; ++k)
        if (k == K) {
          q[k].x = x1 + i * g.dirx;
          q[k].y = y1 + i * g.diry;
        }
      ++K;
    }
    if (fits) {
      const float r2 = p.robot_size * p.robot_size;
      int cnt[KMAX];
      unsigned kmn[KMAX], kmx[KMAX];
#pragma unroll
      for (int k = 0; k < KMAX; ++k) {
        cnt[k] = 0;
        kmn[k] = 0xFFFFFFFFu;
        kmx[k] = 0u;
      }
      switch (K) {
        case 1: sweep_discs<1>(tile, T, q, r2, cnt, kmn, kmx); break;
        case 2: sweep_discs<2>(tile, T, q, r2, cnt, kmn, kmx); break;
        case 3: sweep_discs<3>(tile, T, q, r2, cnt, kmn, kmx); break;
        case 4: sweep_discs<4>(tile, T, q, r2, cnt, kmn, kmx); break;
        case 5: sweep_discs<5>(tile, T, q, r2, cnt, kmn, kmx); break;
        case 6: sweep_discs<6>(tile, T, q, r2, cnt, kmn, kmx); break;
        default: break;
      }
      if (TRG_EDGE_STAGE_CUT == 3) {
        o.status = EDGE_SEG + (cnt[0] + cnt[1] + cnt[2] + cnt[3] + cnt[4] + cnt[5] > 1000000) +
                   ((kmn[0] ^ kmn[1] ^ kmn[2] ^ kmn[3] ^ kmn[4] ^ kmn[5] ^ kmx[0] ^ kmx[1] ^ kmx[2] ^
                     kmx[3] ^ kmx[4] ^ kmx[5]) == 12345u);
        return o;
      }
#pragma unroll
      for (int k = 0; k < KMAX; ++k) {
        if (k < K) {
          const int n = cnt[k];
          hits += (unsigned long long)n;
          bool col;
          if (n == 0) {
            col = true;
          } else {
            const unsigned klo = wave_reduce_key<true>(kmn[k]);
            const unsigned khi = wave_reduce_key<false>(kmx[k]);
            int bad = 0;
            if (!(key_float(khi) - key_float(klo) <= p.height_threshold)) {
              int nn = 0;
              for (int base = 0; base < T; base += WAVE) {
                const int i = base + lane;
                bool hit = false;
                float z = 0.0f;
                if (i < T) {
                  const f2 d = tile.xy[i] - q[k];
                  const f2 dd = d * d;
                  z = tile.z[i];
                  hit = dd.x + dd.y <= r2;
                }
                const unsigned long long mask = ballot(hit);
                if (hit) tile.zb[nn + __popcll(mask & lanemask_lt())] = z;
                nn += __popcll(mask);
              }
              wave_lds_sync();
              if (n <= WAVE) {
                const float zl = tile.zb[lane < n ? lane : 0];
                bad = median_count_lanes(zl, n, p.height_threshold, klo, khi);
              } else {
                bad = median_count(tile.zb, n, p.height_threshold);
              }
              wave_lds_sync();
            }
            if (bad == 0)
              col = 0.0f > p.collision_threshold;
            else
              col = (float)bad / (float)n > p.collision_threshold;
          }
          if (col) {
            o.status = EDGE_SEG | g.uncertain;
            o.hits = (int)hits;
            return o;
          }
        }
      }
      EDGE_CUT(4)
      Gathered mo;
      int kept = 0;
      for (int base = 0; base < T; base += WAVE) {
        const int i = base + lane;
        bool keep = false;
        if (i < T) {
          const f2 pt = tile.xy[i];
          keep = ellipse_point(ep, pt.x, pt.y, tile.z[i], mo);
        }
        kept += __popcll(ballot(keep));
      }
      if constexpr (TRG_EDGE_STAGE_CUT == 5 && MODE == GATHER_FULL) {
        o.status = EDGE_SEG + (mo.s_x + mo.s_y + mo.s_z + mo.s_xx + mo.s_xy + mo.s_xz + mo.s_yy +
                                   mo.s_yz + mo.s_zz == 12345.0) + (kept > 100000);
        return o;
      }
      const int in_range = staged_in_range;
      hits += (unsigned long long)in_range;
      o.hits = (int)hits;
      o.n_pts = kept;
      if (in_range == 0) {
        o.status = EDGE_EMPTY | g.uncertain;
        return o;
      }
      if (kept < 3) {
        o.status = EDGE_FEW | g.uncertain;
        return o;
      }
      if constexpr (MODE == GATHER_FULL) reduce_store_moments(tile, mo, rec);
      o.status = EDGE_OK | g.uncertain;
      return o;
    }
  }

  int guard = 0;
  for (float i = 0; MODE != GATHER_MOMENTS && i < g.dist; i += ds) {
    const float qx = x1 + i * g.dirx;
    const float qy = y1 + i * g.diry;
    bool col;
    int n = 0;
    if (T >= 0) {
      col = tile_disc_collides(tile, T, qx, qy, p.robot_size, p.height_threshold,
                               p.collision_threshold, n);
    } else {
      const Disc d =
          disc_query<false>(m, qx, qy, p.robot_size, p.height_threshold, tile.zb, ctr, TCAP);
      n = d.n;
      col = disc_collides(d, p.collision_threshold);
    }
    hits += (unsigned long long)n;
    if (col) {
      o.status = EDGE_SEG | g.uncertain;
      o.hits = (int)hits;
      return o;
    }
    if (++guard > 100000 || !(ds > 0.0f)) break;
  }

  Gathered mo;
  if (T >= 0) {
    for (int i = lane; i < T; i += WAVE) {
      const f2 pt = tile.xy[i];
      ellipse_point(ep, pt.x, pt.y, tile.z[i], mo);
    }
  } else {
    const CellRange cr = cells_for(m, g.cx, g.cy, a);
    for (int cyi = cr.cy0; cyi <= cr.cy1; ++cyi) {
      const int s = m.cell_start[cyi * m.W + cr.cx0];
      const int e = m.cell_start[cyi * m.W + cr.cx1 + 1];
#pragma clang loop unroll(disable)
      for (int i = s + lane; i < e; i += WAVE) ellipse_point(ep, m.x[i], m.y[i], m.z[i], mo);
    }
  }
  const int in_range = (T >= 0) ? staged_in_range : wave_sum(mo.in_range);
  const int kept = wave_sum(mo.kept);
  o.n_pts = kept;
  if constexpr (MODE == GATHER_MOMENTS) {
    reduce_store_moments(tile, mo, rec);
    o.status = EDGE_OK;
    return o;
  }
  hits += (unsigned long long)in_range;
  o.hits = (int)hits;
  if (in_range == 0) {
    o.status = EDGE_EMPTY | g.uncertain;
    return o;
  }
  if (kept < 3) {
    o.status = EDGE_FEW | g.uncertain;
    return o;
  }
  if constexpr (MODE == GATHER_FULL) reduce_store_moments(tile, mo, rec);
  o.status = EDGE_OK | g.uncertain;
  return o;
}

__device__ __forceinline__ void store_mid(float *rec, const EdgeMidOut &o) {
  if (lane_id() == 0) {
    float4 h;
    h.x = __int_as_float(o.status);
    h.y = __int_as_float(o.n_pts);
    h.z = o.dist;
    h.w = __int_as_float(o.hits);
    *(float4 *)rec = h;
  }
}

__device__ __forceinline__ uint32_t fmix32(uint32_t h) {
  h ^= h >> 16;
  h *= 0x85EBCA6Bu;
  h ^= h >> 13;
  h *= 0xC2B2AE35u;
  h ^= h >> 16;
  return h;
}
__device__ __forceinline__ uint32_t sample_hash(uint32_t seed, uint32_t epoch, uint32_t id,
                                                uint32_t trial) {
  uint32_t h = fmix32(seed ^ 0x9E3779B9u);
  h = fmix32(h + epoch * 0x9E3779B9u + 0x7F4A7C15u);
  h = fmix32(h + id * 0x85EBCA6Bu + 0x165667B1u);
  h = fmix32(h + trial * 0xC2B2AE35u + 0x27D4EB2Fu);
  return h;
}


__global__ void k_init_bounds(unsigned *b) {
  if (threadIdx.x == 0) {
    b[0] = 0xFFFFFFFFu;
    b[1] = 0xFFFFFFFFu;
    b[2] = 0u;
    b[3] = 0u;
  }
}

__global__ __launch_bounds__(256) void k_bounds(const float *xyz, size_t n, size_t stride,
                                                unsigned *b) {
  unsigned mnx = 0xFFFFFFFFu, mny = 0xFFFFFFFFu, mxx = 0u, mxy = 0u;
  for (size_t i = (size_t)blockIdx.x * blockDim.x + threadIdx.x; i < n;
       i += (size_t)gridDim.x * blockDim.x) {
    const unsigned kx = float_key(xyz[i * stride]);
    const unsigned ky = float_key(xyz[i * stride + 1]);
    mnx = min(mnx, kx);
    mxx = max(mxx, kx);
    mny = min(mny, ky);
    mxy = max(mxy, ky);
  }
#pragma unroll
  for (int m = 32; m >= 1; m >>= 1) {
    mnx = min(mnx, (unsigned)__shfl_xor((int)mnx, m));
    mny = min(mny, (unsigned)__shfl_xor((int)mny, m));
    mxx = max(mxx, (unsigned)__shfl_xor((int)mxx, m));
    mxy = max(mxy, (unsigned)__shfl_xor((int)mxy, m));
  }
  __shared__ unsigned red[4][4];
  const int w = threadIdx.x >> 6;
  if (lane_id() == 0) {
    red[w][0] = mnx;
    red[w][1] = mny;
    red[w][2] = mxx;
    red[w][3] = mxy;
  }
  __syncthreads();
  if (threadIdx.x == 0) {
    atomicMin(&b[0], min(min(red[0][0], red[1][0]), min(red[2][0], red[3][0])));
    atomicMin(&b[1], min(min(red[0][1], red[1][1]), min(red[2][1], red[3][1])));
    atomicMax(&b[2], max(max(red[0][2], red[1][2]), max(red[2][2], red[3][2])));
    atomicMax(&b[3], max(max(red[0][3], red[1][3]), max(red[2][3], red[3][3])));
  }
}

__global__ __launch_bounds__(256) void k_cell_count(const float *xyz, size_t n, size_t stride,
                                                    float x0, float y0, float inv_g, int W, int H,
                                                    int *cell_of, int *rank, int *counts) {
  for (size_t i = (size_t)blockIdx.x * blockDim.x + threadIdx.x; i < n;
       i += (size_t)gridDim.x * blockDim.x) {
    const int cx = cell_coord(xyz[i * stride], x0, inv_g, W);
    const int cy = cell_coord(xyz[i * stride + 1], y0, inv_g, H);
    const int c = cy * W + cx;
    cell_of[i] = c;
    rank[i] = atomicAdd(&counts[c], 1);
  }
}

// ... 960 lines not shown
```

### trg-planner_amd/csrc/trg_level.inc

```

__device__ __forceinline__ int call_ref(long long at) { return -(int)(at + 2); }
__device__ __forceinline__ long long call_at(const BfsDev &B, long long call_base, int slot) {
  return call_base + (long long)slot * B.cstride;
}
__device__ __forceinline__ long long ref_call(int n2) { return -(long long)n2 - 2; }

__device__ __forceinline__ float cov_entry(const double (&sm)[9], int kept, int e) {
  const double n = (double)kept;
  const double inv = 1.0 / (double)(kept - 1);
  const double sa = e < 3 ? sm[0] : (e < 5 ? sm[1] : sm[2]);
  const double sb = e == 0 ? sm[0] : ((e == 1 || e == 3) ? sm[1] : sm[2]);
  const double sab = e == 0 ? sm[3] : e == 1 ? sm[4] : e == 2 ? sm[5] : e == 3 ? sm[6] : e == 4 ? sm[7] : sm[8];
  const double ma = sa / n, mb = sb / n;
  return (float)((sab - n * ma * mb) * inv);
}

#ifndef LV_WAVES_PER_SIMD
#define LV_WAVES_PER_SIMD 5
#endif
constexpr int LV_SMAX = 64;
constexpr int LV_NODE_CAP = 256;
#ifndef TRG_LSW
#define TRG_LSW 4
#endif
constexpr int LSW = TRG_LSW;
static_assert(LSW <= SW, "the sampling LDS (SampleLds) is sized for SW waves");
constexpr int LV_WIN_MAX = LSW >= 8 ? 22 : (LSW >= 4 ? 16 : 11);

#ifdef LV_PHASE_TIMING_RESOLVE
#define RV_PHASE(n)                                                                               \
  if (threadIdx.x == 0) {                                                                         \
    const long long now_ = clock64();                                                             \
    atomicAdd(&B.stats64[16 + (blockIdx.x & 1023) * 8 + (n)], (unsigned long long)(now_ - phase_t_)); \
    phase_t_ = clock64();                                                                         \
  }
#define RV_PHASE_BEGIN long long phase_t_ = clock64();
#else
#define RV_PHASE(n)
#define RV_PHASE_BEGIN
#endif
#if defined(LV_PHASE_TIMING) && !defined(LV_PHASE_TIMING_RESOLVE)
#define LV_PHASE(n)                                                                               \
  if (threadIdx.x == 0) {                                                                         \
    const long long now_ = clock64();                                                             \
    atomicAdd(&B.stats64[16 + (blockIdx.x & 1023) * 8 + (n)], (unsigned long long)(now_ - phase_t_)); \
    phase_t_ = clock64();                                                                         \
  }
#define LV_PHASE_BEGIN long long phase_t_ = clock64();
#else
#define LV_PHASE(n)
#define LV_PHASE_BEGIN
#endif

constexpr int TL_UNITS = 1 << 16, TL_KINDS = 12, TL_TAGS = 6;
constexpr size_t TL_STRIDE = (size_t)TL_UNITS * TL_KINDS;
#ifdef LV_TIMELINE
#define TL_MARK(tag, kind, unit)                                                                      \
  do {                                                                                                \
    const unsigned tlt_ = (unsigned)((tag) - (LV_TIMELINE));                                          \
    if (B.tl && tlt_ < (unsigned)TL_TAGS && (unsigned)(unit) < (unsigned)TL_UNITS)                    \
      B.tl[(size_t)tlt_ * TL_STRIDE + (size_t)(kind) * TL_UNITS + (unit)] = (unsigned long long)wall_clock64(); \
  } while (0)
#else
#define TL_MARK(tag, kind, unit)
#endif
struct LevelLds {
  float nd_x[LV_NODE_CAP], nd_y[LV_NODE_CAP];
  int nd_id[LV_NODE_CAP];
  int nd_n;
  int cand[LV_SMAX];
};

__device__ __forceinline__ unsigned long long lv_entry(int tag, int cell) {
  return ((unsigned long long)(unsigned)tag << 32) | (unsigned)cell;
}


template <bool IS_MIN>
__device__ __forceinline__ unsigned half_reduce_key(unsigned v) {
  const unsigned ident = IS_MIN ? 0xFFFFFFFFu : 0u;
#define HKEY_STEP(ctrl, rowmask)                                                                 \
  {                                                                                              \
    const unsigned o = (unsigned)__builtin_amdgcn_update_dpp((int)ident, (int)v, ctrl, rowmask,  \
                                                             0xf, false);                        \
    v = IS_MIN ? (o < v ? o : v) : (o > v ? o : v);                                              \
  }
  HKEY_STEP(0x111, 0xf)
  HKEY_STEP(0x112, 0xf)
  HKEY_STEP(0x114, 0xf)
  HKEY_STEP(0x118, 0xf)
  HKEY_STEP(0x142, 0xa)
#undef HKEY_STEP
  const unsigned r0 = (unsigned)__builtin_amdgcn_readlane((int)v, 31);
  const unsigned r1 = (unsigned)__builtin_amdgcn_readlane((int)v, 63);
  return (lane_id() & 32) ? r1 : r0;
}

__device__ __forceinline__ unsigned half_bits(unsigned long long mask) {
  return (lane_id() & 32) ? (unsigned)(mask >> 32) : (unsigned)mask;
}

struct Disc2 {
  int n, cnt;
  float nn_z, nn_d2;
  int nn_tie;
};

constexpr unsigned long long hsort_keep_min_mask(int K, int J) {
  unsigned long long m = 0;
  for (int l = 0; l < 64; ++l) {
    const int l32 = l & 31;
    if (((l32 & K) == 0) == ((l32 & J) == 0)) m |= 1ull << l;
  }
  return m;
}

__device__ Disc2 sample_tile_disc2(const MapView &m, const SampleLds &L, float *zb, float qx, float qy,
                                   float r, float h) {
  const int lane = lane_id();
  const int hh = lane >> 5, l32 = lane & 31;
  float *zbh = zb + hh * (SHCAP / 2);
  const float r2 = r * r;
  const CellRange c = cells_for(m, qx, qy, r);
  const int cx0 = max(c.cx0 - L.bx0, 0), cx1 = min(c.cx1 - L.bx0, L.ncols - 1);
  const int cy0 = max(c.cy0 - L.by0, 0), cy1 = min(c.cy1 - L.by0, L.nrows - 1);
  const int nrows = cy1 - cy0 + 1;
  const int nrows_max = max(__builtin_amdgcn_readlane(nrows, 0), __builtin_amdgcn_readlane(nrows, 32));
  int n = 0;
  float best_d2 = FLT_MAX, best_z = 0.0f;
  int best_perm = INT_MAX;
  bool lane_tie = false;
  for (int ri = 0; ri < nrows_max; ++ri) {
    const bool rvalid = ri < nrows && cx1 >= cx0;
    const int row = rvalid ? cy0 + ri : 0;
    const int s = rvalid ? L.cs[row][cx0] : 0, e = rvalid ? L.cs[row][cx1 + 1] : 0;
    const int len = e - s;
    const int len_max = max(__builtin_amdgcn_readlane(len, 0), __builtin_amdgcn_readlane(len, 32));
    for (int base = 0; base < len_max; base += 32) {
      const int i = s + base + l32;
      const bool act = base + l32 < len;
      bool hit = false;
      float z = 0.0f, d2 = 0.0f;
      if (act) {
        const f2 pt = L.xy[i];
        const float dx = pt.x - qx;
        const float dy = pt.y - qy;
        z = L.z[i];
        d2 = dx * dx + dy * dy;
        hit = d2 <= r2;
      }
      const unsigned hm = half_bits(ballot(hit));
      if (hit) {
        const int pos = n + __popc(hm & ((1u << l32) - 1u));
        if (pos < SHCAP / 2) zbh[pos] = z;
        const int pm = L.perm[i];
        if (d2 == best_d2) lane_tie = true;
        if (d2 < best_d2) lane_tie = false;
        if (d2 < best_d2 || (d2 == best_d2 && pm < best_perm)) {
          best_d2 = d2;
          best_z = z;
          best_perm = pm;
        }
      }
      n += __popc(hm);
    }
  }
  Disc2 out;
  out.n = n;
  out.cnt = 0;
  out.nn_z = 0.0f;
  out.nn_d2 = 0.0f;
  out.nn_tie = 0;
  const unsigned dkey = __float_as_uint(best_d2);
  const unsigned wdk = half_reduce_key<true>(dkey);
  const bool holds = best_perm != INT_MAX && dkey == wdk;
  const unsigned wp = half_reduce_key<true>(holds ? (unsigned)best_perm : 0xFFFFFFFFu);
  const unsigned who = half_bits(ballot(holds && (unsigned)best_perm == wp));
  const int src = (lane & 32) + (who ? __ffs((int)who) - 1 : 0);
  out.nn_z = __shfl(best_z, src);
  out.nn_d2 = __uint_as_float(wdk);
  out.nn_tie = half_bits(ballot(holds && ((unsigned)best_perm != wp || lane_tie))) != 0u;
  if (n > SHCAP / 2) out.cnt = -1;
  wave_lds_sync();
  const int nq = min(n, SHCAP / 2);
  const float zl = zbh[l32 < nq ? l32 : 0];
  unsigned kmn = 0xFFFFFFFFu, kmx = 0u;
  for (int i = l32; i < nq; i += 32) {
    const unsigned zk = float_key(i == l32 ? zl : zbh[i]);
    kmn = zk < kmn ? zk : kmn;
    kmx = zk > kmx ? zk : kmx;
  }
  const unsigned klo = half_reduce_key<true>(kmn), khi = half_reduce_key<false>(kmx);
  const bool need = n > 0 && out.cnt == 0 && !(key_float(khi) - key_float(klo) <= h);
  const unsigned long long need_m = ballot(need);
  if (need_m) {
    const bool need0 = (need_m & 1ull) != 0ull, need1 = (need_m >> 32) != 0ull;
    const int n0 = __builtin_amdgcn_readlane(n, 0), n1 = __builtin_amdgcn_readlane(n, 32);
    if ((need0 && n0 > 32) || (need1 && n1 > 32)) {
      int c0 = 0, c1 = 0;
      if (need0) c0 = median_count(zb, n0, h);
      if (need1) c1 = median_count(zb + SHCAP / 2, n1, h);
      out.cnt = need ? ((lane & 32) ? c1 : c0) : out.cnt;
    } else {
      float v = (l32 < n) ? zl : FLT_MAX;
#define HSORT_STEP(K, J)                                                                               \
  {                                                                                                    \
    const float o = __int_as_float(__builtin_amdgcn_ds_swizzle(__float_as_int(v), 0x1F | ((J) << 10))); \
    float mn, mx;                                                                                      \
    asm("v_min_f32 %0, %1, %2" : "=v"(mn) : "v"(v), "v"(o));                                           \
    asm("v_max_f32 %0, %1, %2" : "=v"(mx) : "v"(v), "v"(o));                                           \
    asm("v_cndmask_b32 %0, %1, %2, %3" : "=v"(v) : "v"(mx), "v"(mn), "s"(hsort_keep_min_mask(K, J)));  \
  }
      HSORT_STEP(2, 1)
      HSORT_STEP(4, 2) HSORT_STEP(4, 1)
      HSORT_STEP(8, 4) HSORT_STEP(8, 2) HSORT_STEP(8, 1)
      HSORT_STEP(16, 8) HSORT_STEP(16, 4) HSORT_STEP(16, 2) HSORT_STEP(16, 1)
      HSORT_STEP(32, 16) HSORT_STEP(32, 8) HSORT_STEP(32, 4) HSORT_STEP(32, 2) HSORT_STEP(32, 1)
#undef HSORT_STEP
      const float zmed = __shfl(v, (lane & 32) + (n >> 1));
      const unsigned bad = half_bits(ballot(need && l32 < n && fabsf(zl - zmed) > h));
      out.cnt = need ? __popc(bad) : out.cnt;
    }
  }
  wave_lds_sync();
  return out;
}

template <int NW>
struct PureLds {
  float sx[LV_SMAX], sy[LV_SMAX], sz[LV_SMAX];
  int r_col[2][2 * NW];
  unsigned long long r_hits[NW];
  int r_ties[NW];
};

template <int NW>
__device__ __forceinline__ bool sample_pure_stage(const MapView &m, const QueryParams &p, float px, float py,
                                                  SampleLds &L, PureLds<NW> &P) {
  static_assert(NW <= SW, "the sampling LDS (SampleLds) is sized for SW waves");
  if (threadIdx.x < NW) P.r_ties[threadIdx.x] = 0;
  return stage_sample_tile(m, p, px, py, L);
}

template <int NW>
__device__ __forceinline__ void sample_pure_draws(const MapView &m, const QueryParams &p, const float *cos_t,
                                                  const float *sin_t, int table_bits, uint32_t seed, uint32_t epoch,
                                                  const BfsDev &B, int mt_parity, int mt_slot_base,
                                                  DeviceCounters *ctr, uint32_t id, float px, float py, bool use_tile,
                                                  SampleLds &L, PureLds<NW> &P, int &n_acc_out, int &draws_out) {
  const int tid = threadIdx.x;
  const int w = tid >> 6;
  const int lane = lane_id();
  const int S = p.sample_num;
  constexpr int drr = 2 * NW;
  const int max_trial_sample = 1000;
  int n_acc = 0, rejects = 0, draws = 0, round = 0;
  unsigned long long hits = 0;
  const int wu = __builtin_amdgcn_readfirstlane(w);
  const int hh = lane >> 5;
  float c_next, s_next;
  {
    const uint32_t k = sample_hash(seed, epoch, id, (uint32_t)(2 * w + hh)) >> (32 - table_bits);
    c_next = cos_t[k];
    s_next = sin_t[k];
  }
  while (n_acc < S && rejects <= max_trial_sample) {
    const float qx = px + p.expand_dist * c_next;
    const float qy = py + p.expand_dist * s_next;
    {
      const uint32_t k = sample_hash(seed, epoch, id, (uint32_t)(draws + drr + 2 * w + hh)) >> (32 - table_bits);
      c_next = cos_t[k];
      s_next = sin_t[k];
    }
    Disc2 d;
    d.n = 0;
    d.cnt = -1;
    d.nn_z = d.nn_d2 = 0.0f;
    d.nn_tie = 0;
    const bool wave_active = 2 * wu < drr;
    if (wave_active && use_tile) d = sample_tile_disc2(m, L, L.zb[w], qx, qy, p.robot_size, p.height_threshold);
    const unsigned long long slow = wave_active ? ballot(d.cnt < 0) : 0ull;
    if (slow) {
#pragma unroll
      for (int g = 0; g < 2; ++g) {
        if (!((slow >> (32 * g)) & 1ull)) continue;
        const float gx = __shfl(qx, 32 * g), gy = __shfl(qy, 32 * g);
        const Disc dg = disc_query<true>(m, gx, gy, p.robot_size, p.height_threshold, L.zb[w], ctr, SHCAP);
        if (hh == g) {
          d.n = dg.n;
          d.cnt = dg.cnt;
          d.nn_z = dg.nn_z;
          d.nn_d2 = dg.nn_d2;
          d.nn_tie = dg.nn_tie;
        }
      }
    }
    const bool in_core = qx >= p.core_x0 && qx < p.core_x1 && qy >= p.core_y0 && qy < p.core_y1;
    bool collides = true;
    if (ballot(d.n > 0 && d.cnt != 0) != 0ull) {
      if (d.n > 0) collides = (float)d.cnt / (float)d.n > p.collision_threshold;
    } else if (d.n > 0) {
      collides = 0.0f > p.collision_threshold;
    }
    collides = collides || !in_core;
    int *colbuf = P.r_col[round & 1];
    if ((lane & 31) == 0 && 2 * w + hh < drr) colbuf[2 * w + hh] = collides ? 1 : 0;
    __syncthreads();
    const unsigned long long colmask = ballot(lane < drr && colbuf[lane < drr ? lane : 0] != 0);
    int my_slot0 = -1, my_slot1 = -1;
    int consumed = 0;
    for (int i = 0; i < drr; ++i) {
      if (n_acc >= S || rejects > max_trial_sample) break;
      draws++;
      consumed++;
      if ((colmask >> i) & 1ull) {
        rejects++;
      } else {
        if (i == 2 * wu) my_slot0 = n_acc;
        if (i == 2 * wu + 1) my_slot1 = n_acc;
        n_acc++;
      }
    }
    {
      const int n0 = __builtin_amdgcn_readlane(d.n, 0), n1 = __builtin_amdgcn_readlane(d.n, 32);
      if (2 * wu < consumed) hits += (unsigned long long)n0;
      if (2 * wu + 1 < consumed) hits += (unsigned long long)n1;
    }
    const int my_slot = hh ? my_slot1 : my_slot0;
    if (my_slot >= 0 && (lane & 31) == 0) {
      P.sx[my_slot] = qx;
      P.sy[my_slot] = qy;
      P.sz[my_slot] = d.nn_z;
      if (d.nn_tie) {
        atomicAdd(&P.r_ties[w], 1);
        const int k = atomicAdd(&B.ctrs[BFS_CTR_NMAPTIE + mt_parity], 1);
        if (k < MAPTIE_CAP) {
          MapTieRec rec;
          rec.slot = mt_slot_base + my_slot;
          rec.qx = qx;
          rec.qy = qy;
          rec.d2 = d.nn_d2;
          B.mt_rec[mt_parity * MAPTIE_CAP + k] = rec;
        }
      }
    }
    round++;
  }
  if (lane == 0) P.r_hits[w] = hits;
  __syncthreads();
  n_acc_out = n_acc;
  draws_out = draws;
}

template <int NW>
struct SampleSide {
  SampleLds L;
  LevelLds V;
  PureLds<NW> P;
};

template <int NW>
__device__ __forceinline__ void sample_body(SampleSide<NW> &SS, const MapView &m, const QueryParams &p, const float *cos_t,
                                            const float *sin_t, int table_bits, uint32_t seed, uint32_t epoch,
                                            const BfsDev &B, int count, const int *count_dev, int node_base,
                                            int parity, int tag, int pub_stamp, DeviceCounters *ctr, int wg) {
  SampleLds &L = SS.L;
  LevelLds &V = SS.V;
  PureLds<NW> &P = SS.P;
  const int node = wg + node_base;
  if (pub_stamp && wg == 0 && threadIdx.x < BFS_CTR_COUNT && B.host_ctrs) {
    int v = __hip_atomic_load(&B.ctrs[threadIdx.x], __ATOMIC_RELAXED, __HIP_MEMORY_SCOPE_AGENT);
    if (threadIdx.x == BFS_CTR_DONE || threadIdx.x == BFS_CTR_COUNT - 1) v = pub_stamp;
    __hip_atomic_store(&B.host_ctrs[threadIdx.x], v, __ATOMIC_RELAXED, __HIP_MEMORY_SCOPE_SYSTEM);
  }
  if (node == 0 && threadIdx.x == 0) B.stats64[STATS64_EXPAND_START] = (unsigned long long)wall_clock64();
  if (count_dev) count = min(count, *count_dev);
  if (node >= count) return;
  const int tid = threadIdx.x;
  const int w = tid >> 6;
  const int lane = lane_id();
  const int S = p.sample_num;
  if (tid == 0) TL_MARK(tag, 0, node);
  const int gid = B.front_cur[node];
  const float2 pxy = B.fxy_cur[node];
  const float px = pxy.x, py = pxy.y, pz = B.nz[gid];
  const uint32_t id = (uint32_t)gid;
  if (tid == 0) {
    V.nd_n = 0;
  }
  LV_PHASE_BEGIN
  int4 gc0 = {0, 0, 0, 0}, gc1 = gc0, gc2 = gc0;
  int gc_y0 = 0;
  {
    const int K = (int)ceilf(p.expand_dist * 2.01f * B.ginv) + 1;
    const int side = 2 * K + 1;
    const int cx = bfs_cell_x(B, px), cy = bfs_cell_y(B, py);
    if (tid < side * side) {
      const int yy = cy - K + tid / side, xx = cx - K + tid % side;
      const float bx = B.gx0 + (float)xx * B.gcell_size, by = B.gy0 + (float)yy * B.gcell_size;
      const float ddx = fmaxf(fmaxf(bx - px, px - (bx + B.gcell_size)), 0.0f);
      const float ddy = fmaxf(fmaxf(by - py, py - (by + B.gcell_size)), 0.0f);
      const float reach = p.expand_dist * 2.02f + 1e-3f;
      if (yy >= 0 && yy < B.GH && xx >= 0 && xx < B.GW && ddx * ddx + ddy * ddy <= reach * reach) {
        const int4 *c = (const int4 *)&B.gcell[yy * B.GW + xx];
        gc0 = c[0];
        gc1 = c[1];
        gc2 = c[2];
        gc_y0 = ((const int *)c)[12];
      }
    }
  }
  int n_acc = 0, draws = 0;
  unsigned long long hits_node = 0;
  int ties_node = 0;
  const bool use_tile = sample_pure_stage<NW>(m, p, px, py, L, P);
  if (!use_tile) __syncthreads();
  LV_PHASE(0)
  {
    const int cnt = min(gc0.x, GRID_SLOTS);
    if (cnt > 0) {
      const int base = atomicAdd(&V.nd_n, cnt);
      const int ids[4] = {gc0.y, gc0.z, gc0.w, gc1.x};
      const int xs[4] = {gc1.y, gc1.z, gc1.w, gc2.x};
      const int ys[4] = {gc2.y, gc2.z, gc2.w, gc_y0};
#pragma unroll
      for (int qi = 0; qi < GRID_SLOTS; ++qi)
        if (qi < cnt && base + qi < LV_NODE_CAP) {
          V.nd_id[base + qi] = ids[qi];
          V.nd_x[base + qi] = __int_as_float(xs[qi]);
          V.nd_y[base + qi] = __int_as_float(ys[qi]);
        }
    }
  }
  LV_PHASE(1)
  sample_pure_draws<NW>(m, p, cos_t, sin_t, table_bits, seed, epoch, B, parity, node * S, ctr, id, px, py, use_tile,
                         L, P, n_acc, draws);
  if (tid == 0)
    for (int i = 0; i < NW; ++i) {
      hits_node += P.r_hits[i];
      ties_node += P.r_ties[i];
    }
  if (tid == 0 && V.nd_n > LV_NODE_CAP) atomicOr(&B.ctrs[BFS_CTR_ERR], BFS_ERR_GRID_OVERFLOW);
  const int hh = lane >> 5;
  LV_PHASE(2)
  const int nd_n = min(V.nd_n, LV_NODE_CAP);
  {
    const int l32 = lane & 31;
    for (int j0 = w; j0 < S; j0 += 2 * NW) {
      const int j = j0 + hh * NW;
      const bool have_slot = j < S;
      const bool acc = have_slot && j < n_acc;
      const int slot = node * S + j;
      float qx = 0.0f, qy = 0.0f;
      unsigned bkey = 0xFFFFFFFFu;
      int bid = -1;
      bool lane_tie = false;
      if (acc) {
        qx = P.sx[j];
        qy = P.sy[j];
        for (int i = l32; i < nd_n; i += 32) {
          const unsigned k = __float_as_uint(bfs_d2(V.nd_x[i], V.nd_y[i], qx, qy));
          const int nid = V.nd_id[i];
          if (k < bkey) {
            bkey = k;
            bid = nid;
            lane_tie = false;
          } else if (k == bkey && nid != bid) {
            lane_tie = true;
          }
        }
      }
      const unsigned mk = half_reduce_key<true>(bkey);
      const unsigned who = half_bits(ballot(bkey == mk));
      const unsigned tl = half_bits(ballot(bkey == mk && lane_tie));
      int cls = 0, nn = -1;
      float d2 = FLT_MAX;
      const int src = (lane & 32) + (who ? __ffs((int)who) - 1 : 0);
      const int nn_s = __shfl(bid, src);
      if (acc) {
        bool tie = false;
        if (mk != 0xFFFFFFFFu) {
          nn = nn_s;
          d2 = __uint_as_float(mk);
          tie = __popc(who) > 1 || tl != 0u;
          if (tie && l32 == 0) atomicOr(&B.ctrs[BFS_CTR_ERR], BFS_ERR_TIE_CLS);
        }
        cls = ((nn >= 0 && sqrtf(d2) < p.robot_size) ? 1 : 2) | (tie ? SLOT_TIE : 0);
      }
      if (l32 == 0 && have_slot) {
        float4 *rec = (float4 *)&B.slot_rec[slot];
        rec[0] = make_float4(qx, qy, acc ? P.sz[j] : 0.0f, d2);
        rec[1] = make_float4(__int_as_float(nn), __int_as_float(cls), __int_as_float(EDGE_GATE), 0.0f);
        B.c_outcome[slot] = 0;
        V.cand[j] = cls & SLOT_CLS_MASK;
      }
    }
  }
  __syncthreads();
  LV_PHASE(3)
  const unsigned long long cand_mask = ballot(lane < S && V.cand[lane < S ? lane : 0] == 2);
  LV_PHASE(4)
  if (tid == 0) {
    int4 *nr = (int4 *)&B.node_rec[node];
    nr[0] = make_int4(n_acc, draws, (int)hits_node, 0);
    nr[1] = make_int4((int)(unsigned)cand_mask, (int)(unsigned)(cand_mask >> 32), 0, 0);
    ((float4 *)nr)[2] = make_float4(px, py, pz, 0.0f);
    if (ties_node && ctr) atomicAdd(&ctr[wg % COUNTER_SHARDS].nn_ties, (unsigned long long)ties_node);
    TL_MARK(tag, 1, node);
  }
  LV_PHASE(5)
}

template <int NW>
__global__ __launch_bounds__(NW *WAVE, NW == LSW ? LV_WAVES_PER_SIMD : 4) void k_level_sample(
    MapView m, QueryParams p, const float *cos_t, const float *sin_t, int table_bits, uint32_t seed,
    uint32_t epoch, BfsDev B, int count, const int *count_dev, int node_base, int parity, int tag,
    int pub_stamp, DeviceCounters *ctr) {
  __shared__ SampleSide<NW> SS;
  sample_body<NW>(SS, m, p, cos_t, sin_t, table_bits, seed, epoch, B, count, count_dev, node_base, parity, tag,
                  pub_stamp, ctr, (int)blockIdx.x);
}


#ifndef TRG_LQW
#define TRG_LQW 1
#endif
constexpr int LQW = TRG_LQW;
__device__ __forceinline__ bool level_hash_insert(const BfsDev &B, int tag, int slot, float qx, float qy) {
  static_assert(sizeof(HashEnt) == 32, "the table is addressed as 8 words per entry: cell, tag, slot, -, x, y, -, -");
  bool placed = true;
  if (lane_id() == 0) {
    int *tab = (int *)B.lv_hash;
    const uint32_t mask = (uint32_t)B.ht_size - 1u;
    const int key = bfs_cell_y(B, qy) * B.GW + bfs_cell_x(B, qx);
    uint32_t e = bfs_hash(key) & mask;
    placed = false;
    for (uint32_t probe = 0; probe <= mask; ++probe) {
      int *w = tab + 8 * (size_t)e;
      if (atomicMax(&w[1], tag) < tag) {
        w[0] = key;
        w[2] = slot;
        w[4] = __float_as_int(qx);
        w[5] = __float_as_int(qy);
        placed = true;
        break;
      }
      e = (e + 1) & mask;
    }
  }
  return placed;
}

__device__ __forceinline__ void spec_one(const MapView &m, const QueryParams &p, const BfsDev &B, int slot, int node,
                                         int unit, float4 par, float qx, float qy, float qz, WaveTile &tile,
                                         int parity, DeviceCounters *ctr, int tl_tag) {
  const int lane = lane_id();
  if (lane == 0) TL_MARK(tl_tag, 2, unit);
  const EdgeMidOut o = edge_gather<GATHER_STATUS>(m, p, par.x, par.y, par.z, qx, qy, qz, tile, nullptr, ctr);
  float *out = (float *)&B.slot_rec[slot];
  if (lane == 0) {
    out[6] = __int_as_float(o.status);
    out[7] = o.dist;
    out[14] = __int_as_float(0);
    out[15] = __int_as_float(o.hits);
    TL_MARK(tl_tag, 3, unit);
    if (o.hits) atomicAdd(&B.node_rec[node].hits_spec, o.hits);
    if (o.status & EDGE_GATE_UNCERTAIN) {
      const int q = atomicAdd(&B.ctrs[parity ? BFS_CTR_NUNC1 : BFS_CTR_NUNC], 1);
      if (q < BFS_UNC_CAP) {
        const int at = parity * BFS_UNC_CAP + q;
        B.unc_list[at] = slot;
        B.unc_rec[3 * at] = par.z;
        B.unc_rec[3 * at + 1] = qz;
        B.unc_rec[3 * at + 2] = o.dist;
      }
    }
  }
}

__global__ __launch_bounds__(LQW *WAVE, SPEC_WAVES_PER_SIMD) void k_level_spec(MapView m, QueryParams p, BfsDev B,
                                                                            int count, const int *count_dev,
                                                                            int node_base, int parity,
                                                                            DeviceCounters *ctr, int tl_tag) {
  __shared__ WaveTile tiles[LQW];
  const int w = threadIdx.x >> 6;
  const int S = p.sample_num;
  if (count_dev) count = min(count, *count_dev);
  const int slot = node_base * S + blockIdx.x * LQW + w;
  if (slot >= count * S) return;
  const int node = slot / S;
  const int2 cm = *(const int2 *)&B.node_rec[node].cand_lo;
  const float4 r0 = ((const float4 *)&B.slot_rec[slot])[0];
  const float4 par = ((const float4 *)&B.node_rec[node])[2];
  const int j = slot - node * S;
  if (!(((j < 32 ? (unsigned)cm.x : (unsigned)cm.y) >> (j & 31)) & 1u)) return;
  const float sqx = __int_as_float(__builtin_amdgcn_readfirstlane(__float_as_int(r0.x)));
  const float sqy = __int_as_float(__builtin_amdgcn_readfirstlane(__float_as_int(r0.y)));
  spec_one(m, p, B, slot, node, slot - node_base * S, par, r0.x, r0.y, r0.z, tiles[w], parity, ctr, tl_tag);
  if (!level_hash_insert(B, tl_tag, slot, sqx, sqy)) atomicOr(&B.ctrs[BFS_CTR_ERR], BFS_ERR_HASH);
}


#ifndef TRG_POLL_FREE
#define TRG_POLL_FREE 2
#endif
#ifndef TRG_POLL_SLEEP
#define TRG_POLL_SLEEP 2
#endif
constexpr int RG = 4;
constexpr int RWV = TRG_RWV;
static_assert(RWV * RG == RW, "slots per resolve workgroup");
constexpr int NBL = 4;
constexpr int NB_ROW = 16 * NBL;

struct ResolveLds {
  int so[RW];
  int nb_n[RWV][RG];
  int nb_c[RWV][RG][NB_ROW];
  float nb_d[RWV][RG][NB_ROW];
  int spin_max[RWV];
  int c_flag[RW];
  int c_cell[RW];
};
static_assert(RW <= WAVE, "the first wave commits one slot per lane");

__device__ __forceinline__ unsigned row_min_key(unsigned v) {
#define RKEY_STEP(ctrl)                                                                            \
  {                                                                                                \
    const unsigned o = (unsigned)__builtin_amdgcn_update_dpp((int)0xFFFFFFFFu, (int)v, ctrl, 0xf, 0xf, \
                                                             false);                               \
    v = o < v ? o : v;                                                                             \
  }
  RKEY_STEP(0x111)
  RKEY_STEP(0x112)
  RKEY_STEP(0x114)
  RKEY_STEP(0x118)
#undef RKEY_STEP
  return (unsigned)__shfl((int)v, (lane_id() & 48) | 15);
}

#ifndef RESOLVE_WAVES_PER_SIMD
#define RESOLVE_WAVES_PER_SIMD 6
#endif
// ... 270 lines not shown
            if ((st[q] & BL_OPEN) && dd[q] > best) st[q] &= ~BL_OPEN;
            any_open |= (st[q] & BL_OPEN) != 0;
            any_risky |= (st[q] & BL_OPEN) != 0 && (!(sqrtf(dd[q]) >= r) || (st[q] & BL_BAD) != 0);
          }
        }
        const bool wait_exact = ((ballot(any_open) >> rshift) & 0xFFFFull) != 0ull;
        const bool wait_create = ((ballot(any_risky) >> rshift) & 0xFFFFull) != 0ull;
        const bool near = exists && sqrtf(best) < r;
        const bool best_valid = bestc >= 0 ? best_outcome == 3 : nn_valid;
        const bool new_ok = own_ok || (STEP3 && (pre_rescue || ((ballot(rescued) >> rshift) & 0xFFFFull) != 0ull));
        if (!announced && near) {
          if (l16 == 0) {
            vso[slot - wg_base] = 7;
            outcome_store(&B.c_outcome[slot], 7);
          }
          announced = true;
        }
        if (!wait_exact && !last_pass) {
          car_key = mkey;
          car_c = bestc;
          car_o = best_outcome;
          car_tie = tie;
          pdone = true;
        } else if (!wait_exact) {
          if (tie && l16 == 0) report_tie(B, slot);
          if (exists && !best_valid) {
            outcome = 1;
          } else if (near) {
            outcome = 2;
            target = bestc >= 0 ? call_ref(call_at(B, call_base, bestc)) : nn;
          } else {
            outcome = new_ok ? 3 : 4;
          }
        } else if (RESOLVE_EARLY_CREATE && K == 1 && is_cand && !wait_create && !near && (!exists || best_valid) &&
                   !tie) {
          outcome = new_ok ? 3 : 4;
        }
        if (outcome) {
          if (is_cand && l16 == 0) {
            vso[slot - wg_base] = outcome;
            outcome_store(&B.c_outcome[slot], outcome);
          }
          done = true;
          pdone = true;
        }
      }
    }
    if (!MULTI) break;
    ++pass;
    need_probe = !done && cls != 0 && pass < K;
    if (ballot(need_probe) == 0ull || spin >= max_spin) break;
  }
  RV_PHASE(1)
  if (threadIdx.x == 0) TL_MARK(tag + 1, 6, bid);
  if (cls != 0 && outcome == 0 && l16 == 0) atomicOr(&B.ctrs[BFS_CTR_ERR], BFS_ERR_STALL);
  if (slot < slots && l16 == 0) {
    int n2 = -1, st = CALL_NONE;
    float wgt = 0.0f, dist = 0.0f;
    if (outcome == 2) {
      n2 = target;
      st = CALL_PENDING;
    } else if (outcome == 3) {
      n2 = call_ref(call_at(B, call_base, slot));
      st = own_st & EDGE_STATUS_MASK;
      dist = own_dist;
    }
    const size_t at = (size_t)call_at(B, call_base, slot);
    B.call_n1[at] = u;
    B.call_n2[at] = n2;
    B.call_status[at] = (n2 == u) ? CALL_NONE : st;
    B.call_w[at] = wgt;
    B.call_dist[at] = dist;
  } else if (slot < slots && l16 < B.cstride) {
    B.call_status[(size_t)call_at(B, call_base, slot) + l16] = CALL_NONE;
  }
  const bool created = is_cand && (outcome == 3 || outcome == 4) && l16 == 0;
  const bool valid = is_cand && outcome == 3 && l16 == 0;
  if (slot < slots && l16 == 0) {
    const int ls = w * RG + g;
    if (slot % S == 0) {
      const int4 nr = *(const int4 *)&B.node_rec[slot / S];
      const NodeRec &full = B.node_rec[slot / S];
      const int ncand = __popc(full.cand_lo) + __popc(full.cand_hi);
      *(int4 *)&B.nexp[u] = make_int4(nr.x | (ncand << 8), nr.y, nr.z, nr.w);
    }
    if (created) {
      const int cell = bfs_cell_y(B, qy) * B.GW + bfs_cell_x(B, qx);
      GridCell &c = B.gcell[cell];
      const int pos = atomicAdd(&c.cnt, 1);
      if (pos < GRID_SLOTS) {
        c.x[pos] = qx;
        c.y[pos] = qy;
      } else {
        atomicOr(&B.ctrs[BFS_CTR_ERR], BFS_ERR_GRID_OVERFLOW);
      }
      R.c_cell[ls] = pos < GRID_SLOTS ? cell * GRID_SLOTS + pos : -1;
    }
    R.c_flag[ls] = created ? (valid ? 2 : 1) : 0;
  }
  if (lane == 0) R.spin_max[w] = spin;
  RV_PHASE(2)
  __syncthreads();
  if (w != 0) return;
  RV_PHASE(3)
  const int flag = lane < RW ? R.c_flag[lane] : 0;
  const unsigned long long cb = ballot(flag != 0), vb = ballot(flag == 2);
  int sm = 0;
  for (int i = 0; i < RWV; ++i) sm = max(sm, R.spin_max[i]);
  const unsigned long long ep = (unsigned long long)(unsigned)epoch & 0xFFFFFull;
  if (lane < RW && wg_base + lane < slots)
    __hip_atomic_store(&B.c_cell[wg_base + lane],
                       (ep << 44) | ((unsigned long long)(unsigned)flag << 42) | (unsigned)(flag ? R.c_cell[lane] : 0),
                       __ATOMIC_RELAXED, __HIP_MEMORY_SCOPE_AGENT);
  if (lane == 0) {
    const unsigned long long own_c = (unsigned long long)__popcll(cb), own_v = (unsigned long long)__popcll(vb);
    __hip_atomic_store(&B.wg_state[bid], (ep << 44) | (1ull << 42) | (own_c << 21) | own_v, __ATOMIC_RELAXED,
                       __HIP_MEMORY_SCOPE_AGENT);
    if (sm > 0) atomicMax(&B.stats64[6], (unsigned long long)sm);
    TL_MARK(tag + 1, 7, bid);
  }
  RV_PHASE(4)
}

constexpr int CRW = RWV * WAVE / RW;
struct CommitLds {
  int red_c[RWV], red_v[RWV];
  int pre_c[CRW + 1], pre_v[CRW + 1];
  int failed;
};
__device__ __forceinline__ void commit_role(CommitLds &C, const BfsDev &B, int m, int S, long long call_base,
                                            int stall_test, int max_spin, int V0, int new_state, int epoch, int c,
                                            int nR, int nC, int tl_tag) {
  const int tid = threadIdx.x, lane = lane_id(), w = tid >> 6;
  const int slots = m * S;
  if (tid == 0) TL_MARK(tl_tag, 10, c);
  const int first = c * CRW, last = min(first + CRW, nR);
  const unsigned long long ep = (unsigned long long)(unsigned)epoch & 0xFFFFFull;
  if (tid <= CRW) {
    C.pre_c[tid] = 0;
    C.pre_v[tid] = 0;
  }
  if (tid == 0) C.failed = (stall_test == 2 && c == nC / 2) ? 1 : 0;
  __syncthreads();
  const int slot = first * RW + tid;
  int flag = 0, cp = -1;
  if (slot < slots) {
    long long polls = 0;
    for (;;) {
      const unsigned long long fc = __hip_atomic_load(&B.c_cell[slot], __ATOMIC_RELAXED, __HIP_MEMORY_SCOPE_AGENT);
      if ((fc >> 44) == ep) {
        flag = (int)((fc >> 42) & 3ull);
        cp = (int)(unsigned)fc;
        break;
      }
      if (++polls > 64ll * max_spin) {
        atomicOr(&B.ctrs[BFS_CTR_ERR], BFS_ERR_LOOKBACK);
        break;
      }
      __builtin_amdgcn_s_sleep(2);
    }
  }
  float4 r0 = make_float4(0.f, 0.f, 0.f, 0.f);
  int4 s2 = make_int4(0, 0, 0, 0), s3 = s2;
  if (flag != 0) {
    const int4 *src = (const int4 *)&B.slot_rec[slot];
    r0 = ((const float4 *)src)[0];
    s2 = src[2];
    s3 = src[3];
  }
  int sum_c = 0, sum_v = 0;
  for (int i = tid; i < last; i += RWV * WAVE) {
    unsigned long long v = 0;
    long long polls = 0;
    for (;;) {
      v = __hip_atomic_load(&B.wg_state[i], __ATOMIC_RELAXED, __HIP_MEMORY_SCOPE_AGENT);
      if ((v >> 44) == ep && ((v >> 42) & 3ull) != 0ull) break;
      if (++polls > 64ll * max_spin || *(volatile int *)&C.failed) {
        C.failed = 1;
        v = 0;
        break;
      }
      __builtin_amdgcn_s_sleep(4);
    }
    const int cc = (int)((v >> 21) & 0x1FFFFFull), vv = (int)(v & 0x1FFFFFull);
    if (i < first) {
      sum_c += cc;
      sum_v += vv;
    } else {
      C.pre_c[i - first + 1] = cc;
      C.pre_v[i - first + 1] = vv;
    }
  }
  sum_c = wave_sum(sum_c);
  sum_v = wave_sum(sum_v);
  if (lane == 0) {
    C.red_c[w] = sum_c;
    C.red_v[w] = sum_v;
  }
  __syncthreads();
  if (C.failed) {
    if (tid == 0) atomicOr(&B.ctrs[BFS_CTR_ERR], BFS_ERR_LOOKBACK);
    return;
  }
  if (tid == 0) {
    int ac = 0, av = 0;
    for (int i = 0; i < RWV; ++i) {
      ac += C.red_c[i];
      av += C.red_v[i];
    }
    for (int k = 0; k <= CRW; ++k) {
      ac += C.pre_c[k];
      av += C.pre_v[k];
      C.pre_c[k] = ac;
      C.pre_v[k] = av;
    }
    if (c == nC - 1) {
      B.ctrs[BFS_CTR_V] = V0 + C.pre_c[last - first];
      B.ctrs[BFS_CTR_MNEXT] = C.pre_v[last - first];
    }
  }
  __syncthreads();
  if (tid == 0) TL_MARK(tl_tag, 11, c);
  static_assert(WAVE % RW == 0, "a wave of the commit covers whole resolve workgroups");
  const unsigned long long cb = ballot(flag != 0), vb = ballot(flag == 2);
  if (flag == 0) return;
  const unsigned long long gmask = (RW == 64 ? ~0ull : ((1ull << (RW % 64)) - 1ull)) << ((lane / RW) * RW);
  const unsigned long long below = lanemask_lt() & gmask;
  const int k = tid / RW;
  const int before_c = C.pre_c[k] + __popcll(cb & below);
  const int before_v = C.pre_v[k] + __popcll(vb & below);
  const int id = V0 + before_c;
  B.newid_of_call[call_at(B, call_base, slot)] = id;
  if (id < B.vcap) {
    B.nx[id] = r0.x;
    B.ny[id] = r0.y;
    B.nz[id] = r0.z;
    B.nstate[id] = flag == 2 ? new_state : -1;
    B.nhits[id] = s3.w;
    if (flag == 2) {
      int4 *dst = (int4 *)&B.ncov[id];
      dst[0] = s2;
      dst[1] = make_int4(s3.x, s3.y, s3.z, (int)call_at(B, call_base, slot));
    }
    if (cp >= 0) B.gcell[cp / GRID_SLOTS].id[cp % GRID_SLOTS] = id;
  } else {
    atomicOr(&B.ctrs[BFS_CTR_ERR], BFS_ERR_VCAP);
  }
  if (flag == 2) {
    if (before_v < B.fcap) {
      B.front_next[before_v] = id;
      B.fxy_next[before_v] = make_float2(r0.x, r0.y);
    } else {
      atomicOr(&B.ctrs[BFS_CTR_ERR], BFS_ERR_LEVEL_TOO_BIG);
    }
  }
}

template <bool TICKET, bool MULTI, bool STEP3>
__global__ __launch_bounds__(RWV *WAVE, (MULTI || STEP3) ? RESOLVE_WAVES_PER_SIMD : RESOLVE_WAVES_PER_SIMD_PLAIN) void k_level_resolve(
    BfsDev B, int m, int S, float d, float r, int tag, long long call_base, int stall_test, int max_spin, int V0,
    int new_state, int epoch, int nR, int nC, unsigned ticket_base) {
  __shared__ union {
    ResolveLds R;
    CommitLds C;
  } sh;
  __shared__ int wg_ticket;
  int bid = (int)blockIdx.x;
  if (TICKET) {
    if (threadIdx.x == 0) wg_ticket = (int)(atomicAdd(B.ticket, 1u) - ticket_base);
    __syncthreads();
    bid = wg_ticket;
  }
  if (bid >= nR + nC) return;
  if (bid == 0 && threadIdx.x == 0) {
    const unsigned long long t0 = B.stats64[STATS64_EXPAND_START];
    if (t0) {
      B.stats64[STATS64_EXPAND_TICKS] += (unsigned long long)wall_clock64() - t0;
      B.stats64[STATS64_EXPAND_START] = 0ull;
    }
  }
  if (bid >= nR) {
    commit_role(sh.C, B, m, S, call_base, stall_test, max_spin, V0, new_state, epoch, bid - nR, nR, nC, tag + 1);
  } else {
    resolve_body<MULTI, STEP3>(sh.R, B, m, S, d, r, tag, call_base, stall_test, max_spin, V0, new_state, epoch, bid, nR);
  }
}

__global__ __launch_bounds__(256) void k_bfs_stats(BfsDev B, int V, unsigned long long *out) {
  __shared__ unsigned long long red[6][4];
  unsigned long long a[6] = {0, 0, 0, 0, 0, 0};
  for (int id = blockIdx.x * 256 + threadIdx.x; id < V; id += gridDim.x * 256) {
    if (B.nstate[id] != -1) {
      const int4 n = *(const int4 *)&B.nexp[id];
      a[0] += (unsigned long long)n.y;
      a[1] += (unsigned long long)(n.x & 0xFF);
      a[2] += (unsigned long long)n.z;
      a[3] += (unsigned long long)n.w;
      a[4] += (unsigned long long)((n.x >> 8) & 0x3FFFFF);
    }
    if (id > 0) a[5] += (unsigned long long)B.nhits[id];
  }
#pragma unroll
  for (int q = 0; q < 6; ++q) {
#pragma unroll
    for (int msk = 32; msk >= 1; msk >>= 1) a[q] += __shfl_xor(a[q], msk);
    if (lane_id() == 0) red[q][threadIdx.x >> 6] = a[q];
  }
  __syncthreads();
  if (threadIdx.x < 6) {
    const unsigned long long t = red[threadIdx.x][0] + red[threadIdx.x][1] + red[threadIdx.x][2] + red[threadIdx.x][3];
    if (t) atomicAdd(&out[threadIdx.x], t);
  }
}

constexpr int NCW = 4;
__global__ __launch_bounds__(NCW *WAVE, EDGE_WAVES_PER_SIMD) void k_node_cov(MapView m, QueryParams p, BfsDev B, int v_lo,
                                                                          int v_hi) {
  __shared__ WaveTile tiles[NCW];
  __shared__ alignas(16) float mids[NCW][MID_STRIDE];
  const int w = threadIdx.x >> 6, lane = lane_id();
  const int id = v_lo + blockIdx.x * NCW + w;
  if (id < 1 || id >= min(v_hi, B.vcap) || B.nstate[id] == -1) return;
  const int2 gc = *(const int2 *)&B.ncov[id].w_given;
  if (gc.x) return;
  const size_t at = (size_t)gc.y;
  const int st = B.call_status[at];
  if (st < 0 || (st & EDGE_STATUS_MASK) != EDGE_OK) return;
  const int par = B.call_n1[at];
  float *rec = mids[w];
  const EdgeMidOut o = edge_gather<GATHER_MOMENTS>(m, p, B.nx[par], B.ny[par], B.nz[par], B.nx[id], B.ny[id],
                                                   B.nz[id], tiles[w], rec, nullptr);
  wave_lds_sync();
  if (lane < 6) {
    double sm[9];
    const double *src = (const double *)(rec + MID_MOMENTS);
#pragma unroll
    for (int i = 0; i < 9; ++i) sm[i] = src[i];
    B.ncov[id].cov[lane] = cov_entry(sm, o.n_pts, lane);
  }
}

__global__ __launch_bounds__(256) void k_node_weights(BfsDev B, int V) {
  const int id = 1 + blockIdx.x * blockDim.x + threadIdx.x;
  if (id >= V || B.nstate[id] == -1) return;
  const NodeCov nc = B.ncov[id];
  const size_t at = (size_t)nc.call;
  int st = B.call_status[at];
  if (st < 0 || (st & EDGE_STATUS_MASK) != EDGE_OK) return;
  float w;
  if (nc.w_given) {
    w = nc.cov[0];
  } else {
    float cov[3][3];
    cov[0][0] = nc.cov[0];
    cov[0][1] = cov[1][0] = nc.cov[1];
    cov[0][2] = cov[2][0] = nc.cov[2];
    cov[1][1] = nc.cov[3];
    cov[1][2] = cov[2][1] = nc.cov[4];
    cov[2][2] = nc.cov[5];
    int clamped = 0;
    w = risk_weight(cov, clamped);
    st |= clamped;
  }
  B.call_w[at] = w;
  B.call_status[at] = st;
}
```

### trg-planner_amd/trg_planner/_engine.py

```python
from __future__ import annotations

import ctypes as C
import os
import subprocess

import numpy as np

_HERE = os.path.dirname(os.path.abspath(__file__))
CSRC = os.path.normpath(os.path.join(_HERE, "..", "csrc"))
LIB_PATH = os.environ.get("TRG_ENGINE_LIB") or os.path.join(CSRC, "libtrg_engine.so")

KIND_GLOBAL, KIND_LOCAL, KIND_PRECLEAN, KIND_STITCHED = 0, 1, 2, 3
_KINDS = {"global": KIND_GLOBAL, "local": KIND_LOCAL, "preclean": KIND_PRECLEAN,
          "stitched": KIND_STITCHED}

STATUS_NAMES = {0: "TRG_OK", 1: "TRG_ERR_INVALID_ARG", 2: "TRG_ERR_NO_MAP", 3: "TRG_ERR_NO_ROOT",
                4: "TRG_ERR_DEVICE", 5: "TRG_ERR_NO_GRAPH", 6: "TRG_ERR_NOT_FOUND",
                7: "TRG_ERR_IO", 8: "TRG_ERR_CAPACITY"}


class TrgError(RuntimeError):
    def __init__(self, status, message):
        super().__init__(f"{STATUS_NAMES.get(status, status)}: {message}")
        self.status = status


class TrgParams(C.Structure):
    _fields_ = [("is_verbose", C.c_int32), ("expand_dist", C.c_float), ("robot_size", C.c_float),
                ("sample_num", C.c_int32), ("height_threshold", C.c_float),
                ("collision_threshold", C.c_float), ("update_collision_threshold", C.c_float),
                ("safety_factor", C.c_float), ("goal_tolerance", C.c_float)]


class TrgSampler(C.Structure):
    _fields_ = [("seed", C.c_uint32), ("table_bits", C.c_int32)]


class TrgCsrView(C.Structure):
    _fields_ = [("num_nodes", C.c_int32), ("num_edges", C.c_int32),
                ("node_xyz", C.POINTER(C.c_float)), ("node_state", C.POINTER(C.c_int32)),
                ("rowptr", C.POINTER(C.c_int32)), ("col", C.POINTER(C.c_int32)),
                ("weight", C.POINTER(C.c_float)), ("dist", C.POINTER(C.c_float)),
                ("creation_id", C.POINTER(C.c_int32))]


class TrgPathInfo(C.Structure):
    _fields_ = [("direct_dist", C.c_float), ("path_length", C.c_float), ("avg_risk", C.c_float),
                ("num_points", C.c_int32)]


class TrgFieldInfo(C.Structure):
    _fields_ = [("source", C.c_int32), ("reached", C.c_int32), ("rounds", C.c_int32),
                ("host_syncs", C.c_int32), ("ms_device", C.c_double), ("ms_total", C.c_double)]


class TrgTiledFieldInfo(C.Structure):
    _fields_ = [("exchanges", C.c_int32), ("rounds", C.c_int32), ("ghosts", C.c_int32), ("border_nodes", C.c_int32),
                ("records_sent", C.c_int64), ("ms_device", C.c_float), ("ms_total", C.c_float)]


class TrgRouteInfo(C.Structure):
    _fields_ = [("num_nodes", C.c_int32), ("cost", C.c_float), ("path_length", C.c_float),
                ("avg_risk", C.c_float)]


class TrgFieldModel(C.Structure):
    _fields_ = [("safety_factor", C.c_float), ("max_weight", C.c_float)]


class TrgPoseInfo(C.Structure):
    _fields_ = [("status", C.c_int32), ("n_candidates", C.c_int32), ("n_links", C.c_int32), ("z", C.c_float)]


class TrgStats(C.Structure):
    _fields_ = [(n, C.c_uint64) for n in (
        "map_points", "expanded_nodes", "trials", "samples", "created_nodes", "invalid_nodes",
        "edge_calls", "edge_evals_gpu", "nn_ties", "gate_uncertain", "sync_batches",
        "bytes_sample_kernel", "bytes_spec_kernel", "bytes_edge_kernel", "bytes_index_build")] + [
        ("ms_index_build", C.c_double), ("ms_sample_kernel", C.c_double),
        ("ms_spec_kernel", C.c_double), ("ms_edge_kernel", C.c_double),
        ("launches_sample_kernel", C.c_uint64), ("launches_spec_kernel", C.c_uint64),
        ("launches_edge_kernel", C.c_uint64), ("ms_set_map_total", C.c_double),
        ("ms_init_graph_total", C.c_double), ("ms_replay_host", C.c_double),
        ("ms_finalize_host", C.c_double), ("ms_wait_gpu", C.c_double),
        ("bfs_levels", C.c_uint64), ("used_device_bfs", C.c_uint64), ("bfs_fallbacks", C.c_uint64),
        ("bfs_max_spin", C.c_uint64), ("bfs_host_levels", C.c_uint64),
        ("map_nn_ties", C.c_uint64),
        ("ms_bfs_loop", C.c_double), ("ms_deferred", C.c_double),
        ("map_nn_resolved", C.c_uint64), ("map_nn_unresolved", C.c_uint64),
        ("bfs_tie_fixups", C.c_uint64), ("bytes_spec_created", C.c_uint64),
        ("ms_rare_events", C.c_double), ("bfs_ticket_reruns", C.c_uint64),
        ("bfs_multipass_rows", C.c_uint64), ("ms_upload", C.c_double), ("presampled_nodes", C.c_uint64),
        ("stitch_gate_retries", C.c_uint64), ("stitch_regrows", C.c_uint64)]


EXPORTS = [
    "trg_engine_create", "trg_engine_destroy", "trg_engine_last_error", "trg_engine_device_arch",
    "trg_engine_set_global_map", "trg_engine_set_global_map_device", "trg_engine_set_local_map",
    "trg_engine_reset_map", "trg_engine_reset_graph", "trg_engine_init_graph",
    "trg_engine_update_graph", "trg_engine_export_csr", "trg_engine_save_json",
    "trg_engine_load_json", "trg_engine_plan", "trg_engine_refine_path",
    "trg_engine_is_collision_batch", "trg_engine_nearest_z_batch", "trg_engine_edge_risk_batch",
    "trg_engine_is_frontier_batch", "trg_engine_get_stats", "trg_engine_get_sampler_table",
    "trg_engine_debug_map_index", "trg_engine_set_option", "trg_engine_fallback_reason",
    "trg_engine_check_reached", "trg_engine_check_replan", "trg_engine_set_tile",
    "trg_engine_voxel_filter", "trg_engine_plan_batch",
    "trg_engine_stitch_boundary", "trg_engine_stitch_cross", "trg_engine_stitch_assemble",
    "trg_engine_graph_sizes",
    "trg_engine_comm_unique_id", "trg_engine_comm_init", "trg_engine_comm_adopt", "trg_engine_comm_destroy",
    "trg_engine_comm_join_local",
    "trg_engine_stitch_exchange", "trg_engine_cost_field", "trg_engine_cost_field_batch",
    "trg_engine_field_routes", "trg_engine_cost_field_bounded", "trg_engine_field_reached",
    "trg_engine_cost_field_sets", "trg_engine_cost_field_refresh", "trg_engine_cost_field_models",
    "trg_engine_risk_field_sets", "trg_engine_risk_field_refresh",
    "trg_engine_pose_links", "trg_engine_cost_field_seeded",
    "trg_engine_tiled_cost_field", "trg_engine_stitch_ids",
]

TRG_FIELD_BATCH_MAX = 64
SETTLE_NONE, SETTLE_ANY, SETTLE_ALL = 0, 1, 2
_SETTLE = {None: SETTLE_NONE, "any": SETTLE_ANY, "all": SETTLE_ALL}


def build_library(force=False):
    import glob
    srcs = []
    for pat in ("*.hip", "*.inc", "*.ipp", "*.h", "*.cpp", "*.sh"):
        srcs += glob.glob(os.path.join(CSRC, pat))
    srcs += glob.glob(os.path.normpath(os.path.join(CSRC, "..", "..", "include", "*")))
    stale = force or not os.path.exists(LIB_PATH) or not glob.glob(os.path.join(_HERE, "_trg_pybind*.so"))
    if not stale:
        t = os.path.getmtime(LIB_PATH)
        stale = any(os.path.exists(s) and os.path.getmtime(s) > t for s in srcs)
    if stale:
        subprocess.check_call(["bash", os.path.join(CSRC, "build.sh")])
    return LIB_PATH


_lib = None


def load_library():
    global _lib
    if _lib is not None:
        return _lib
    if not os.path.exists(LIB_PATH):
        raise ImportError(f"{LIB_PATH} is missing: run trg-planner_amd/csrc/build.sh "
                          "(__graft_entry__.build()); there is no CPU fallback")
    L = C.CDLL(LIB_PATH)
    fp, ip = C.POINTER(C.c_float), C.POINTER(C.c_int32)
    vp = C.c_void_p
    L.trg_engine_create.argtypes = [C.POINTER(TrgParams), C.c_int, C.POINTER(vp)]
    L.trg_engine_destroy.argtypes = [vp]
    L.trg_engine_destroy.restype = None
    L.trg_engine_last_error.argtypes = [vp]
    L.trg_engine_last_error.restype = C.c_char_p
    L.trg_engine_device_arch.argtypes = [vp]
    L.trg_engine_device_arch.restype = C.c_char_p
    L.trg_engine_set_global_map.argtypes = [vp, fp, C.c_size_t, C.c_size_t]
    L.trg_engine_set_global_map_device.argtypes = [vp, vp, C.c_size_t, C.c_size_t]
    L.trg_engine_set_local_map.argtypes = [vp, fp, fp, C.c_size_t, C.c_size_t]
    L.trg_engine_reset_map.argtypes = [vp, C.c_int]
    L.trg_engine_reset_graph.argtypes = [vp, C.c_int]
    L.trg_engine_init_graph.argtypes = [vp, fp, C.POINTER(TrgSampler)]
    L.trg_engine_update_graph.argtypes = [vp]
    L.trg_engine_export_csr.argtypes = [vp, C.c_int, C.POINTER(TrgCsrView)]
    L.trg_engine_save_json.argtypes = [vp, C.c_char_p]
    L.trg_engine_load_json.argtypes = [vp, C.c_char_p]
    L.trg_engine_plan.argtypes = [vp, fp, fp, fp, C.c_int32, C.POINTER(TrgPathInfo)]
    L.trg_engine_refine_path.argtypes = [fp, C.c_int32, fp, C.c_int32]
    L.trg_engine_refine_path.restype = C.c_int32
    L.trg_engine_plan_batch.argtypes = [vp, fp, fp, C.c_size_t, fp, C.c_int32,
                                        C.POINTER(C.c_int32), C.POINTER(TrgPathInfo)]
    L.trg_engine_voxel_filter.argtypes = [vp, fp, C.c_size_t, C.c_size_t, C.c_float, fp,
                                          C.POINTER(C.c_size_t), C.POINTER(C.c_int32)]
    L.trg_engine_is_collision_batch.argtypes = [vp, C.c_int, C.c_float, fp, C.c_size_t, ip, ip, ip]
# ... 907 lines not shown
```

Baseline: 185.9 million.

## Reuse each node's known start-disc hit count to skip first edge-walk query

Stores each node's disc hit count (ndisc) when it is created and passes it into edge_gather. The edge walk can then start one step past the parent node instead of re-querying the map disc at the edge origin. This removes one disc query per edge evaluation in the speculative and call-gather paths. In exchange it adds a per-node ndisc array with its memset and copies, repacks SlotRec/NodeRec with a narrowed covariance field, adds counters, and lowers the staged-query cap by one when the start is known. It also switches the hit accumulator from 64-bit to 32-bit.

```diff
diff --git a/include/trg_engine.h b/include/trg_engine.h
--- a/include/trg_engine.h
+++ b/include/trg_engine.h
@@ -114,6 +114,7 @@
   uint64_t presampled_nodes;
   uint64_t stitch_gate_retries;
   uint64_t stitch_regrows;
+  uint64_t start_discs_known;
 } TrgStats;
 
 TrgStatus trg_engine_create(const TrgParams *params, int device, TrgEngine **out);
diff --git a/trg-planner_amd/csrc/trg_bfs.inc b/trg-planner_amd/csrc/trg_bfs.inc
--- a/trg-planner_amd/csrc/trg_bfs.inc
+++ b/trg-planner_amd/csrc/trg_bfs.inc
@@ -84,29 +84,38 @@
   if (B.call_status[at] != CALL_PENDING) return;
   const int a = B.call_n1[at], b = B.call_n2[at];
   float *rec = B.mid + (size_t)q * MID_STRIDE;
+  const int n0 = __builtin_amdgcn_readfirstlane(B.ndisc ? B.ndisc[a] : -1);
   const EdgeMidOut o = edge_gather(m, p, B.nx[a], B.ny[a], B.nz[a], B.nx[b], B.ny[b], B.nz[b],
-                                   lds.w[w], rec, ctr);
-  store_mid(rec, o);
+                                   lds.w[w], rec, ctr, n0);
+  store_mid(rec, o, n0);
 }
 
 __global__ __launch_bounds__(256) void k_calls_finish(BfsDev B, const int *list, int count,
                                                       const int *count_dev, DeviceCounters *ctr) {
-  __shared__ int wave_hits[4];
+  __shared__ int wave_hits[4], wave_known[4];
   const int q = blockIdx.x * blockDim.x + threadIdx.x;
   if (count_dev) count = min(count, *count_dev);
   const size_t at = (size_t)list[q < count ? q : 0];
   const bool live = q < count && B.call_status[at] == CALL_PENDING;
   const float *r = B.mid + (size_t)(live ? q : 0) * MID_STRIDE;
+  const int st_word = live ? __float_as_int(r[0]) : 0;
   const int h = wave_sum(live ? __float_as_int(r[MID_HITS]) : 0);
-  if (lane_id() == 0) wave_hits[threadIdx.x >> 6] = h;
+  const int kn = __popcll(ballot((st_word & MID_START_KNOWN) != 0));
+  if (lane_id() == 0) {
+    wave_hits[threadIdx.x >> 6] = h;
+    wave_known[threadIdx.x >> 6] = kn;
+  }
   __syncthreads();
   if (threadIdx.x == 0 && ctr) {
     const unsigned long long tot =
         (unsigned long long)(wave_hits[0] + wave_hits[1] + wave_hits[2] + wave_hits[3]);
     if (tot) atomicAdd(&ctr[blockIdx.x % COUNTER_SHARDS].edge_hits, tot);
+    const unsigned long long tk =
+        (unsigned long long)(wave_known[0] + wave_known[1] + wave_known[2] + wave_known[3]);
+    if (tk) atomicAdd(&ctr[blockIdx.x % COUNTER_SHARDS].start_known, tk);
   }
   if (!live) return;
-  int st = __float_as_int(r[0]);
+  int st = st_word & ~MID_START_KNOWN;
   float w = 0.0f;
   if ((st & EDGE_STATUS_MASK) == EDGE_OK) {
     float cov[3][3];
diff --git a/trg-planner_amd/csrc/trg_engine.cpp b/trg-planner_amd/csrc/trg_engine.cpp
--- a/trg-planner_amd/csrc/trg_engine.cpp
+++ b/trg-planner_amd/csrc/trg_engine.cpp
@@ -541,6 +541,7 @@
   bool keep_preclean = false;
   bool use_device_bfs = true;
   bool defer_overlap = true;
+  bool known_start_disc = true;
   bool tail_overlap = true;
   PlanScratch plan_scratch;
   std::unique_ptr<Uploader> uploader;
@@ -565,6 +566,7 @@
   std::unique_ptr<BfsBuffers> bfs;
   std::string bfs_fallback_reason;
   uint64_t lv_hits_sample = 0, lv_hits_spec = 0;
+  uint64_t lv_start_known = 0;
   TrgStats stats{};
 
   int goal_node = -1;
@@ -1007,7 +1009,7 @@
     e->stats.ms_set_map_total = keep.ms_set_map_total;
   }
   HIPCHK(e, hipMemsetAsync(e->d_ctr, 0, COUNTER_SHARDS * sizeof(DeviceCounters), e->s_main));
-  e->lv_hits_sample = e->lv_hits_spec = 0;
+  e->lv_hits_sample = e->lv_hits_spec = e->lv_start_known = 0;
   if (!e->use_device_bfs) ensure_real_map(e);
   MapOrderSim sim_before;
   if (e->use_device_bfs) {
@@ -1057,7 +1059,7 @@
     HIPCHK(e, hipStreamSynchronize(e->s_main));
     HIPCHK(e, hipStreamSynchronize(e->s_edge));
     HIPCHK(e, hipMemset(e->d_ctr, 0, COUNTER_SHARDS * sizeof(DeviceCounters)));
-    e->lv_hits_sample = e->lv_hits_spec = 0;
+    e->lv_hits_sample = e->lv_hits_spec = e->lv_start_known = 0;
     e->nodes_sim = sim_before;
     ensure_real_map(e);
     reset_graph_global(e);
@@ -1097,6 +1099,7 @@
       {"replay", HOST_OR_DEVICE, &e->use_device_bfs},
       {"defer_overlap", ZERO_OR_ONE, &e->defer_overlap},
       {"tail_overlap", ZERO_OR_ONE, &e->tail_overlap},
+      {"known_start_disc", ZERO_OR_ONE, &e->known_start_disc},
       {"tie_inplace", BOOL, &e->tie_inplace},
       {"keep_preclean", BOOL, &e->keep_preclean},
       {"resolve_tickets", INT, &e->resolve_tickets},
diff --git a/trg-planner_amd/csrc/trg_engine_bfs.inc b/trg-planner_amd/csrc/trg_engine_bfs.inc
--- a/trg-planner_amd/csrc/trg_engine_bfs.inc
+++ b/trg-planner_amd/csrc/trg_engine_bfs.inc
@@ -28,18 +28,19 @@
               "pinned words overlap");
 
 enum : int {
+  S64_SPEC_KNOWN = STATS64_SPEC_KNOWN ,
   S64_DEF_KEPT = 5, S64_MAX_SPIN, S64_MULTIPASS, S64_DRAWS, S64_SAMPLES, S64_DISC_HITS, S64_SPEC_HITS,
   S64_CANDIDATES, S64_PARENT_HITS, S64_EXPAND_START = STATS64_EXPAND_START, S64_EXPAND_TICKS = STATS64_EXPAND_TICKS,
   S64_PHASES = 16, S64_WORDS = 16 + 1024 * 8
 };
-static_assert(S64_PARENT_HITS < S64_EXPAND_START && S64_EXPAND_START < S64_EXPAND_TICKS && S64_EXPAND_TICKS < S64_PHASES,
+static_assert(S64_SPEC_KNOWN < S64_DEF_KEPT && S64_PARENT_HITS < S64_EXPAND_START && S64_EXPAND_START < S64_EXPAND_TICKS && S64_EXPAND_TICKS < S64_PHASES,
               "report_stats fetches the words in front of S64_PHASES");
 
 struct BfsBuffers {
   BfsDev B{};
   FinDev F{};
   LevelSet lv[2];
-  DevArr nx, ny, nz, nstate, gcell, ncov, nexp, nhits, front0, front1, fxy0, fxy1;
+  DevArr nx, ny, nz, nstate, ndisc, gcell, ncov, nexp, nhits, front0, front1, fxy0, fxy1;
   DevArr mid, unc_list, unc_rec, mt_rec, ctrs, stats64, wg_state, c_cell, tl, scan_tmp, s3_scratch;
   DevArr call_n1, call_n2, call_status, call_w, call_dist, newid_of_call, call_slot;
   DevArr sel_list, def_counts;
@@ -550,6 +551,10 @@
     HIPCHK(e, hipMemcpy(B.nstate + at, bb.hm_state.data() + at, n * sizeof(int), hipMemcpyHostToDevice));
     HIPCHK(e, hipMemcpy(B.ncov + at, new_cov.data(), n * sizeof(NodeCov), hipMemcpyHostToDevice));
     HIPCHK(e, hipMemcpy(B.nhits + at, new_hits.data(), n * sizeof(int), hipMemcpyHostToDevice));
+    if (B.ndisc) {
+      const std::vector<int> unknown(n, -1);
+      HIPCHK(e, hipMemcpy(B.ndisc + at, unknown.data(), n * sizeof(int), hipMemcpyHostToDevice));
+    }
     launch_bfs_insert_nodes(B, V0, created, s);
   }
   if (!next_front.empty()) {
@@ -660,6 +665,12 @@
   B.ny = (float *)bb.ny.p;
   B.nz = (float *)bb.nz.p;
   B.nstate = (int *)bb.nstate.p;
+  B.ndisc = nullptr;
+  if (e->known_start_disc) {
+    if ((st = ensure_bytes(e, bb.ndisc, vcap * I)) != TRG_OK) return st;
+    B.ndisc = (int *)bb.ndisc.p;
+    HIPCHK(e, hipMemsetAsync(B.ndisc, 0xFF, vcap * I, s));
+  }
   B.vcap = (int)std::min<size_t>(vcap, 0x7FFFFFF0);
   B.gcell = (GridCell *)bb.gcell.p;
   B.ncov = (NodeCov *)bb.ncov.p;
@@ -1196,6 +1207,7 @@
   e->stats.edge_evals_gpu = s64[S64_CANDIDATES] + s64[S64_DEF_KEPT];
   e->lv_hits_sample = s64[S64_DISC_HITS];
   e->lv_hits_spec = s64[S64_SPEC_HITS];
+  e->lv_start_known = s64[S64_SPEC_KNOWN];
   e->stats.bytes_spec_created = 12ull * s64[S64_PARENT_HITS];
   e->stats.ms_finalize_host = ms_since(t_fin);
   e->stats.bfs_levels = (uint64_t)levels;
diff --git a/trg-planner_amd/csrc/trg_kernels.h b/trg-planner_amd/csrc/trg_kernels.h
--- a/trg-planner_amd/csrc/trg_kernels.h
+++ b/trg-planner_amd/csrc/trg_kernels.h
@@ -60,7 +60,8 @@
   unsigned long long spec_hits;
   unsigned long long nn_ties;
   unsigned long long overflow;
-  unsigned long long pad[11];
+  unsigned long long start_known;
+  unsigned long long pad[10];
 };
 
 void launch_init_bounds(unsigned *d_bounds, hipStream_t s);
@@ -151,7 +152,8 @@
   int cls;
   int status;
   float dist;
-  float cov[6];
+  float cov[5];
+  int ndisc;
   int w_given;
   int hits;
 };
@@ -160,10 +162,12 @@
   int n_acc, n_draws;
   int hits_sample, hits_spec;
   unsigned cand_lo, cand_hi;
-  int pad1[2];
+  int spec_known;
+  int pad1;
   float px, py, pz;
-  int pad2;
-};
+  int pdisc;
+};
+static_assert(sizeof(SlotRec) == 64 && sizeof(NodeRec) == 48, "the level kernels address these records by 16-byte words");
 struct alignas(16) HashEnt {
   unsigned long long tagcell;
   int slot;
@@ -186,6 +190,7 @@
 struct BfsDev {
   float *nx, *ny, *nz;
   int *nstate;
+  int *ndisc;
   NodeCov *ncov;
   int vcap;
   GridCell *gcell;
@@ -220,6 +225,7 @@
   unsigned long long *tl;
 };
 constexpr int STATS64_EXPAND_START = 14, STATS64_EXPAND_TICKS = 15;
+constexpr int STATS64_SPEC_KNOWN = 4;
 
 struct FinDev {
   unsigned long long *ht_key;
diff --git a/trg-planner_amd/csrc/trg_kernels.hip b/trg-planner_amd/csrc/trg_kernels.hip
--- a/trg-planner_amd/csrc/trg_kernels.hip
+++ b/trg-planner_amd/csrc/trg_kernels.hip
@@ -455,6 +455,7 @@
 constexpr int MID_STRIDE = 24;
 constexpr int MID_HITS = 3;
 constexpr int MID_MOMENTS = 4;
+constexpr int MID_START_KNOWN = 1 << 8;
 
 struct EdgeGeom {
   float dist, dirx, diry, cx, cy;
@@ -864,7 +865,7 @@
 template <int MODE = GATHER_FULL>
 __device__ EdgeMidOut edge_gather(const MapView &m, const QueryParams &p, float x1, float y1,
                                   float z1, float x2, float y2, float z2, WaveTile &tile,
-                                  float *rec, DeviceCounters *ctr) {
+                                  float *rec, DeviceCounters *ctr, int n0 = -1) {
   const int lane = lane_id();
   EdgeMidOut o;
   o.n_pts = 0;
@@ -927,8 +928,12 @@
     return o;
   }
 
-  unsigned long long hits = 0;
   const float ds = p.robot_size * 0.5f;
+  const bool known =
+      __builtin_amdgcn_readfirstlane((MODE != GATHER_MOMENTS && n0 >= 0 && 0.0f < g.dist) ? 1 : 0) != 0;
+  unsigned hits = known ? (unsigned)n0 : 0u;
+  const float walk0 = known ? ds : 0.0f;
+  const float wdist = __int_as_float(__builtin_amdgcn_readfirstlane(__float_as_int(g.dist)));
   typedef typename std::conditional<MODE == GATHER_STATUS, EllipseCounts, Moments>::type Gathered;
 
   if (MODE != GATHER_MOMENTS && T >= 0 && ds > 0.0f) {
@@ -937,8 +942,9 @@
     bool fits = true;
 #pragma unroll
     for (int k = 0; k < KMAX; ++k) q[k] = f2{0.0f, 0.0f};
-    for (float i = 0; i < g.dist; i += ds) {
-      if (K == KMAX) {
+    const int kcap = known ? KMAX - 1 : KMAX;
+    for (float i = walk0; i < wdist; i += ds) {
+      if (K == kcap) {
         fits = false;
         break;
       }
@@ -979,7 +985,7 @@
       for (int k = 0; k < KMAX; ++k) {
         if (k < K) {
           const int n = cnt[k];
-          hits += (unsigned long long)n;
+          hits += (unsigned)n;
           bool col;
           if (n == 0) {
             col = true;
@@ -1042,7 +1048,7 @@
         return o;
       }
       const int in_range = staged_in_range;
-      hits += (unsigned long long)in_range;
+      hits += (unsigned)in_range;
       o.hits = (int)hits;
       o.n_pts = kept;
       if (in_range == 0) {
@@ -1060,7 +1066,7 @@
   }
 
   int guard = 0;
-  for (float i = 0; MODE != GATHER_MOMENTS && i < g.dist; i += ds) {
+  for (float i = walk0; MODE != GATHER_MOMENTS && i < wdist; i += ds) {
     const float qx = x1 + i * g.dirx;
     const float qy = y1 + i * g.diry;
     bool col;
@@ -1074,7 +1080,7 @@
       n = d.n;
       col = disc_collides(d, p.collision_threshold);
     }
-    hits += (unsigned long long)n;
+    hits += (unsigned)n;
     if (col) {
       o.status = EDGE_SEG | g.uncertain;
       o.hits = (int)hits;
@@ -1106,7 +1112,7 @@
     o.status = EDGE_OK;
     return o;
   }
-  hits += (unsigned long long)in_range;
+  hits += (unsigned)in_range;
   o.hits = (int)hits;
   if (in_range == 0) {
     o.status = EDGE_EMPTY | g.uncertain;
@@ -1121,10 +1127,14 @@
   return o;
 }
 
-__device__ __forceinline__ void store_mid(float *rec, const EdgeMidOut &o) {
+__device__ __forceinline__ bool edge_start_known(const EdgeMidOut &o, int n0) {
+  return n0 >= 0 && 0.0f < o.dist && (o.status & EDGE_STATUS_MASK) != EDGE_GATE;
+}
+
+__device__ __forceinline__ void store_mid(float *rec, const EdgeMidOut &o, int n0 = -1) {
   if (lane_id() == 0) {
     float4 h;
-    h.x = __int_as_float(o.status);
+    h.x = __int_as_float(o.status | (edge_start_known(o, n0) ? MID_START_KNOWN : 0));
     h.y = __int_as_float(o.n_pts);
     h.z = o.dist;
     h.w = __int_as_float(o.hits);
diff --git a/trg-planner_amd/csrc/trg_level.inc b/trg-planner_amd/csrc/trg_level.inc
--- a/trg-planner_amd/csrc/trg_level.inc
+++ b/trg-planner_amd/csrc/trg_level.inc
@@ -68,6 +68,7 @@
   float nd_x[LV_NODE_CAP], nd_y[LV_NODE_CAP];
   int nd_id[LV_NODE_CAP];
   int nd_n;
+  int pdisc;
   int cand[LV_SMAX];
 };
 
@@ -229,6 +230,7 @@
 template <int NW>
 struct PureLds {
   float sx[LV_SMAX], sy[LV_SMAX], sz[LV_SMAX];
+  int sn[LV_SMAX];
   int r_col[2][2 * NW];
   unsigned long long r_hits[NW];
   int r_ties[NW];
@@ -331,6 +333,7 @@
       P.sx[my_slot] = qx;
       P.sy[my_slot] = qy;
       P.sz[my_slot] = d.nn_z;
+      P.sn[my_slot] = d.n;
       if (d.nn_tie) {
         atomicAdd(&P.r_ties[w], 1);
         const int k = atomicAdd(&B.ctrs[BFS_CTR_NMAPTIE + mt_parity], 1);
@@ -384,6 +387,7 @@
   const int gid = B.front_cur[node];
   const float2 pxy = B.fxy_cur[node];
   const float px = pxy.x, py = pxy.y, pz = B.nz[gid];
+  if (tid == 0) V.pdisc = B.ndisc ? B.ndisc[gid] : -1;
   const uint32_t id = (uint32_t)gid;
   if (tid == 0) {
     V.nd_n = 0;
@@ -491,6 +495,7 @@
         float4 *rec = (float4 *)&B.slot_rec[slot];
         rec[0] = make_float4(qx, qy, acc ? P.sz[j] : 0.0f, d2);
         rec[1] = make_float4(__int_as_float(nn), __int_as_float(cls), __int_as_float(EDGE_GATE), 0.0f);
+        if ((cls & SLOT_CLS_MASK) == 2) B.slot_rec[slot].ndisc = P.sn[j];
         B.c_outcome[slot] = 0;
         V.cand[j] = cls & SLOT_CLS_MASK;
       }
@@ -504,7 +509,7 @@
     int4 *nr = (int4 *)&B.node_rec[node];
     nr[0] = make_int4(n_acc, draws, (int)hits_node, 0);
     nr[1] = make_int4((int)(unsigned)cand_mask, (int)(unsigned)(cand_mask >> 32), 0, 0);
-    ((float4 *)nr)[2] = make_float4(px, py, pz, 0.0f);
+    ((float4 *)nr)[2] = make_float4(px, py, pz, __int_as_float(V.pdisc));
     if (ties_node && ctr) atomicAdd(&ctr[wg % COUNTER_SHARDS].nn_ties, (unsigned long long)ties_node);
     TL_MARK(tag, 1, node);
   }
@@ -556,9 +561,11 @@
                                          int parity, DeviceCounters *ctr, int tl_tag) {
   const int lane = lane_id();
   if (lane == 0) TL_MARK(tl_tag, 2, unit);
-  const EdgeMidOut o = edge_gather<GATHER_STATUS>(m, p, par.x, par.y, par.z, qx, qy, qz, tile, nullptr, ctr);
+  const int n0 = __builtin_amdgcn_readfirstlane(__float_as_int(par.w));
+  const EdgeMidOut o = edge_gather<GATHER_STATUS>(m, p, par.x, par.y, par.z, qx, qy, qz, tile, nullptr, ctr, n0);
   float *out = (float *)&B.slot_rec[slot];
   if (lane == 0) {
+    if (edge_start_known(o, n0)) atomicAdd(&B.node_rec[node].spec_known, 1);
     out[6] = __int_as_float(o.status);
     out[7] = o.dist;
     out[14] = __int_as_float(0);
@@ -995,7 +1002,7 @@
       const int4 nr = *(const int4 *)&B.node_rec[slot / S];
       const NodeRec &full = B.node_rec[slot / S];
       const int ncand = __popc(full.cand_lo) + __popc(full.cand_hi);
-      *(int4 *)&B.nexp[u] = make_int4(nr.x | (ncand << 8), nr.y, nr.z, nr.w);
+      *(int4 *)&B.nexp[u] = make_int4(nr.x | (ncand << 8) | (full.spec_known << 16), nr.y, nr.z, nr.w);
     }
     if (created) {
       const int cell = bfs_cell_y(B, qy) * B.GW + bfs_cell_x(B, qx);
@@ -1150,6 +1157,7 @@
     B.nz[id] = r0.z;
     B.nstate[id] = flag == 2 ? new_state : -1;
     B.nhits[id] = s3.w;
+    if (B.ndisc) B.ndisc[id] = s3.y;
     if (flag == 2) {
       int4 *dst = (int4 *)&B.ncov[id];
       dst[0] = s2;
@@ -1199,9 +1207,10 @@
   }
 }
 
+constexpr int BFS_STATS_N = 7;
 __global__ __launch_bounds__(256) void k_bfs_stats(BfsDev B, int V, unsigned long long *out) {
-  __shared__ unsigned long long red[6][4];
-  unsigned long long a[6] = {0, 0, 0, 0, 0, 0};
+  __shared__ unsigned long long red[BFS_STATS_N][4];
+  unsigned long long a[BFS_STATS_N] = {0, 0, 0, 0, 0, 0, 0};
   for (int id = blockIdx.x * 256 + threadIdx.x; id < V; id += gridDim.x * 256) {
     if (B.nstate[id] != -1) {
       const int4 n = *(const int4 *)&B.nexp[id];
@@ -1209,20 +1218,23 @@
       a[1] += (unsigned long long)(n.x & 0xFF);
       a[2] += (unsigned long long)n.z;
       a[3] += (unsigned long long)n.w;
-      a[4] += (unsigned long long)((n.x >> 8) & 0x3FFFFF);
+      a[4] += (unsigned long long)((n.x >> 8) & 0xFF);
+      a[6] += (unsigned long long)((n.x >> 16) & 0xFF);
     }
     if (id > 0) a[5] += (unsigned long long)B.nhits[id];
   }
 #pragma unroll
-  for (int q = 0; q < 6; ++q) {
+  for (int q = 0; q < BFS_STATS_N; ++q) {
 #pragma unroll
     for (int msk = 32; msk >= 1; msk >>= 1) a[q] += __shfl_xor(a[q], msk);
     if (lane_id() == 0) red[q][threadIdx.x >> 6] = a[q];
   }
   __syncthreads();
-  if (threadIdx.x < 6) {
+  if (threadIdx.x < BFS_STATS_N) {
     const unsigned long long t = red[threadIdx.x][0] + red[threadIdx.x][1] + red[threadIdx.x][2] + red[threadIdx.x][3];
-    if (t) atomicAdd(&out[threadIdx.x], t);
+    unsigned long long *const dst[BFS_STATS_N] = {&out[0], &out[1], &out[2], &out[3], &out[4], &out[5],
+                                                  &B.stats64[STATS64_SPEC_KNOWN]};
+    if (t) atomicAdd(dst[threadIdx.x], t);
   }
 }
 
diff --git a/trg-planner_amd/trg_planner/_engine.py b/trg-planner_amd/trg_planner/_engine.py
--- a/trg-planner_amd/trg_planner/_engine.py
+++ b/trg-planner_amd/trg_planner/_engine.py
@@ -91,7 +91,8 @@
         ("bfs_tie_fixups", C.c_uint64), ("bytes_spec_created", C.c_uint64),
         ("ms_rare_events", C.c_double), ("bfs_ticket_reruns", C.c_uint64),
         ("bfs_multipass_rows", C.c_uint64), ("ms_upload", C.c_double), ("presampled_nodes", C.c_uint64),
-        ("stitch_gate_retries", C.c_uint64), ("stitch_regrows", C.c_uint64)]
+        ("stitch_gate_retries", C.c_uint64), ("stitch_regrows", C.c_uint64),
+        ("start_discs_known", C.c_uint64)]
 
 
 EXPORTS = [
```

After: 187.9 million, median of 6. +1.1%, better.
